# Chain123/RecGURU

Hardware: AMD Instinct MI355X
Metric: user-sequences/sec (AE+GAN step) (higher is better)
Workload: dtype bf16; 1 GPU; cross-domain RecGURU AE+GAN phase-2 iteration (5 critic + 1 generator update), two 100000-item domains; per_gpu_batch=4096, seq_len=200, d_model=128, n_head=4, n_blocks=3, d_ff=512, n_negs=30, user_lengths=U{5..220}, parallelism=dp1

## Files before the change

### include/recguru_hip.h

```cpp
#ifndef RECGURU_HIP_H
#define RECGURU_HIP_H
#include <stddef.h>
#include <stdint.h>
#ifdef __cplusplus
extern "C" {
#endif

#define RG_F32 0
#define RG_BF16 1
#define RG_X3 2

#define RG_ERR_INVALID (-1)
#define RG_ERR_UNSUPPORTED (-2)
#define RG_ERR_HIP (-3)

const char* rg_last_error(void);
int rg_version(void);

int rg_det_enabled(void);
int rg_det_set_arenas(void* fbase0, void* sbase0, unsigned long long bytes0, int bits0,
                      void* fbase1, void* sbase1, unsigned long long bytes1, int bits1);
int rg_det_fault(int clear);

#define RG_PRO_NONE 0
// ... 33 lines not shown
  const void* Y; int ldy;
  const void* X; int ldx;
  float* dW; int lddw;
  float* colsum;
  int T, N1, N2;
  int prologue_x;
  float scale;
  int splits;
  int use_tr;
  const int* live16;
  float* partials;
  int colsum_T;
} rg_gemm_tn_args;
int rg_gemm_tn(const rg_gemm_tn_args* args , int dtype, void* stream);
size_t rg_gemm_tn_workspace(const rg_gemm_tn_args* args , int dtype);
int rg_gemm_tn_layer_supported(const rg_gemm_tn_args* p , const int* wgs , int dtype);
size_t rg_gemm_tn_layer_workspace(int slot, int wgs);
int rg_gemm_tn_layer(const rg_gemm_tn_args* p , const int* wgs , int dtype, void* stream);
int rg_gemm_nt_plan(const rg_gemm_nt_args* args , int dtype, char* name, int cap);
int rg_gemm_tn_plan(const rg_gemm_tn_args* args , int dtype, char* name, int cap);


typedef struct {
  const void* qkv;
  const int64_t* key_ids; int64_t pad_value; int causal;
  void* ctx; float* lse;
  int B, L, H, dk;
  float scale;
  float drop_p; unsigned long long seed;
  const float* rowmask;
  const void* x; const void* wqkv; const float* bqkv; int d;
  int x_masked;
  const int* first_live;
  int qkv_hm;
  const void* pad_rows;
} rg_attn_args;
int rg_attn_fwd(const rg_attn_args* args , int dtype, void* stream);
int rg_attn_fwd_x_supported(int d, int dtype, float drop_p);

typedef struct {
  const void* qkv; const void* dctx; const void* ctx; const float* lse;
  const int64_t* key_ids; int64_t pad_value; int causal;
  void* dqkv;
  int B, L, H, dk;
  float scale;
  float drop_p; unsigned long long seed;
  const float* rowmask;
  const float* bqkv; int x_masked;
  const int* first_live;
  int qkv_hm;
} rg_attn_bwd_args;
int rg_attn_bwd(const rg_attn_bwd_args* args , int dtype, void* stream);

int rg_embed_pe_fwd(const void* table, const float* pe, const int64_t* ids, const float* mask, void* out,
                    long long ntok, int L, int d, float drop_p, unsigned long long seed, int dtype, void* stream);
int rg_embed_pe_fwd_rows(const void* table, long long table_rows, const float* pe, const int64_t* ids, const float* mask, void* out,
                         long long ntok, int L, int d, float drop_p, unsigned long long seed, int dtype, void* stream);
int rg_embed_pe_fwd2(const void* table, const float* pe, const int64_t* ids, const float* mask, void* out, void* out2,
                     long long ntok, int L, int d, float drop_p, unsigned long long seed, int dtype, void* stream);
int rg_embed_pe_fwd_split(const float* table_f32, const float* pe, const int64_t* ids, const float* mask, void* out,
                          void* out_lo, long long ntok, int L, int d, float drop_p, unsigned long long seed, void* stream);
int rg_embed_scatter_bwd(const void* dx, const int64_t* ids, const float* mask, float* dE, long long ntok, int d,
                         long long skip_row, float drop_p, unsigned long long seed, int dtype, void* stream);
size_t rg_embed_scatter_binned_workspace(long long ntok, int d, long long table_rows);
int rg_embed_scatter_bwd_binned(const void* dx, const int64_t* ids, const float* mask, float* dE, long long ntok, int d,
                                long long table_rows, long long skip_row, float drop_p, unsigned long long seed,
                                void* workspace, size_t workspace_bytes, int dtype, void* stream);

typedef struct {
  const void* dy; const void* y; const float* rstd; const float* gamma; const float* beta;
  const float* rowmask;
  void* dz; float* dgamma; float* dbeta;
  long long M; int N; int ld;
  void* dz_drop; float drop_p; unsigned long long drop_seed;
  const int* live16;
  float* dz_colsum;
  float* partials;
} rg_ln_bwd_args;
int rg_ln_bwd(const rg_ln_bwd_args* args , int dtype, void* stream);
size_t rg_ln_bwd_workspace(long long M, int N);

int rg_bcast_add_ln(const void* x, const float* o, const float* gamma, const float* beta, void* y, float* rstd,
                    long long M, int L, int N, float eps, int dtype, void* stream);
int rg_seq_sum(const void* x, void* out , int B, int L, int N, int dtype, void* stream);
int rg_pad_mask(const int64_t* ids, int64_t pad, float* out, long long n, void* stream);
int rg_last_rows(const void* x, const float* rowmask, void* x_last, float* m_last, int B, int L, int d, int dtype, void* stream);

int rg_colsum(const void* x, const void* aux , const float* coef , float* out,
              long long M, int N, int ld, float scale, int dtype,
              void* stream);
int rg_outer_posmask(const float* coef , const float* w , const void* aux, void* out,
                     long long M, int N, float scale, int dtype,
                     void* stream);
typedef struct {
  const void* real; const void* fake;
  const float* alpha;
  const void *W1, *W2, *W3, *W1t, *W2t, *W3t;
  const float *b1, *b2, *b3, *w4, *b4;
  int B, d, n1, n2, n3;
  float drop_p;
  unsigned long long seed_w[3];
  unsigned long long seed_g[3];
  float coef_real, coef_fake;
  float gp_coef;
  float* out;
  float* scalars;
  void *Y1, *X1, *Y2, *X2, *Y3, *X3;
  float *db1, *db2, *db3, *dw4, *db4;
  void* dx;
  void* hscratch;
  int need_wgrad;
  int debug_ablate;
  long long* stamps;
} rg_disc_args;
int rg_disc_supported(int d, int n1, int n2, int n3, int dtype);
int rg_disc_rows(const rg_disc_args* args , int dtype, void* stream);
int rg_interpolate(const float* alpha, const void* real, const void* fake, void* out, long long B, int d,
                   int dtype, void* stream);
int rg_gp_penalty(const float* g, void* dg, float* gp, long long B, int d, float lambda, int dtype,
                  void* stream);
int rg_sum(const float* x, float* out, long long n, float scale, void* stream);

int rg_adam(float* p, const float* g, float* m, float* v, void* shadow, int shadow_dtype, long long n, float lr,
            float beta1, float beta2, float eps, int step, void* stream);
typedef struct {
  float* p; const float* g; float* m; float* v;
  long long n;
  float step_lr; float inv_bc2_sqrt;
} rg_adam_seg;
int rg_adam_multi(const rg_adam_seg* segs , int nsegs, float beta1, float beta2, float eps, void* stream);
typedef struct {
  float* p; const float* g; float* m; float* v;
  long long n;
  long long step;
} rg_adam_seg_dev;
int rg_adam_multi_dev(rg_adam_seg_dev* segs , int nsegs, double lr, double beta1, double beta2,
                      double eps, void* stream);
typedef struct {
  double total_sq;
  float norm;
  float coef;
  int skip;
  int reserved;
  long long skipped;
} rg_adam_ctl;
#define RG_SQNORM_CHAIN(chunk, nsegs) \
  (((chunk) + 1023) / 1024 + 1 + 2 + 6 + 2 + 1 + (int)(((((long long)(nsegs)) + 255) / 256 + 8) >> 29))
int rg_grad_sqnorm_multi(const rg_adam_seg_dev* segs , int nsegs, float* partial ,
                         rg_adam_ctl* ctl , double max_norm, int skip_nonfinite, void* stream);
int rg_adam_multi_dev2(rg_adam_seg_dev* segs , int nsegs, double lr, double beta1, double beta2,
                       double eps, double weight_decay, int decoupled, const rg_adam_ctl* ctl , void* stream);
#define RG_CAST_TRANSPOSE 1
#define RG_CAST_PACK 2
#define RG_CAST_SPLIT 4
int rg_cast(const float* src, void* dst, int R, int C, int transpose, int dtype, void* stream);
typedef struct {
  const float* src; void* dst;
  int R, C, ld, row_off, col_off, transpose;
} rg_cast_seg;
int rg_cast_multi(const rg_cast_seg* segs , const int* tiles , int ntiles,
                  int dtype, void* stream);

#define RG_LOSS_SAMPLED_CE 0
#define RG_LOSS_BPR 1
#define RG_LOSS_BPR_SAS 2
typedef struct {
  const void* h;
// ... 94 lines not shown

typedef struct {
  const void* h;
  const void* table;
  long long first_row, n_rows;
  const int64_t* target;
  const int64_t* excl;
  const int64_t* excl_off;
  int64_t* topk_ids;
  float* topk_scores;
  int* rank;
  void* workspace; size_t workspace_bytes;
  int B, d, K;
} rg_topk_args;
size_t rg_topk_workspace(int B, int d, long long n_rows, int K);
int rg_topk_scores(const rg_topk_args* args , int dtype, void* stream);

typedef struct {
  const void* h;
  const void* table;
  long long table_rows;
  const int64_t* rows;
  long long n_list;
  const int64_t* target;
  const int64_t* excl;
  const int64_t* excl_off;
  int64_t* topk_ids;
  float* topk_scores;
  int* rank;
  void* workspace; size_t workspace_bytes;
  int B, d, K;
} rg_topk_list_args;
size_t rg_topk_list_workspace(int B, int d, long long n_list, int K);
int rg_topk_list(const rg_topk_list_args* args , int dtype, void* stream);

typedef struct {
  const void* ctx; const void* x;
  const void* Wo; const float* bo; const float* g1; const float* be1;
  const float* o_bcast; const float* gc; const float* bec; int L;
  const void* W1; const float* b1; const void* W2; const float* b2; const float* g2; const float* be2;
  const float* rowmask;
  void* out;
  void* y_save; float* rstd1; void* y2_save; float* rstd_c; void* h1_save; float* rstd2;
  int M, d, P, dff; float eps;
  float drop_p; unsigned long long seed_h1; unsigned long long seed_out;
  const float* cross_s; const float* cross_oh; const float* cross_bo; int H;
  const int* live16;
  int skip_dead_saves;
  int w_packed;
  const void* x_lo;
  void* out_lo;
} rg_post_attn_args;
int rg_post_attn_fwd(const rg_post_attn_args* args , int dtype, void* stream);

typedef struct {
  const void* dl2;
  const void* dz;
  const void* h1;
  const void* W2t;
  const void* W1t;
  void* dh1;
  void* dy;
  int M, d, dff, w_packed;
  float nz_scale;
  const int* live16;
  const void* ln_dout; const void* ln_out; const float* ln_rstd; const float* ln_gamma; const float* ln_beta;
  const float* ln_rowmask;
  void* dl2_out; float* ln_dgamma; float* ln_dbeta; float* ln_partials;
  float ln_drop_p; unsigned long long ln_drop_seed;
} rg_ffn_bwd_args;
size_t rg_ffn_bwd_ln_workspace(int M);

typedef struct {
  const void* dy; const void* y; const float* rstd; const float* gamma; const float* beta;
  const float* rowmask;
  const void* Wot;
  void* dz; void* dctx;
  float* dgamma; float* dbeta; float* ln_partials;
  int M, d, P, w_packed;
  const int* live16;
} rg_attn_out_bwd_args;
int rg_attn_out_bwd(const rg_attn_out_bwd_args* args , int dtype, void* stream);
size_t rg_attn_out_bwd_workspace(int M);
int rg_ffn_bwd_data(const rg_ffn_bwd_args* args , int dtype, void* stream);
int rg_ffn_bwd_data_supported(int d, int dff);
int rg_live_tiles(const float* rowmask, long long M, int* list, void* stream);
int rg_first_live(const float* rowmask, int B, int L, int* first, void* stream);

int rg_attn_lastq_fwd(const void* qlast, const void* kv, const int64_t* key_ids, int64_t pad_value, void* ctx,
                      int B, int L, int H, float scale, float drop_p, unsigned long long seed, int dtype, void* stream,
                      const float* bkv, const int* first_live);
int rg_attn_lastq_bwd(const void* qlast, const void* kv, const void* dctx, const int64_t* key_ids, int64_t pad_value,
                      void* dq, void* dkv, int B, int L, int H, float scale, float drop_p, unsigned long long seed,
                      int dtype, void* stream, const float* bkv, const int* first_live);

typedef struct {
  const void* x; const void* qlast; const void* wk; const void* wv;
  const float* bk; const float* bv;
  const int64_t* key_ids; int64_t pad_value;
  const int* first_live;
  void* ctx;
  const void* dctx;
  void* dx; void* dq; void* ym_v; void* ym_q; void* xbar; void* dqp; float* dbv;
  int B, L; float scale; float drop_p; unsigned long long seed;
} rg_lastq_x_args;
int rg_attn_lastq_x_supported(int d, int P, int H, int L, int dtype);
int rg_attn_lastq_x_fwd(const rg_lastq_x_args* args , void* stream);
int rg_attn_lastq_x_bwd(const rg_lastq_x_args* args , void* stream);
int rg_attn_lastq_xf_fwd(const rg_lastq_x_args* args , void* stream);
int rg_attn_lastq_xf_bwd(const rg_lastq_x_args* args , void* stream);

int rg_cross_drop_scale(const int64_t* enc_ids, int64_t pad_value, float* s, int B, int L, int H, float drop_p,
                        unsigned long long seed, void* stream);
int rg_seq_wsum(const void* x, const float* s, void* out, int B, int L, int H, int N, int dtype, void* stream);

#ifdef __cplusplus
}
#endif
#endif
```

### recguru_amd/csrc/elementwise.hip

```cpp
#include <stdlib.h>
#include "rg_common.hip.h"
#include "rg_det.hip.h"
#include "../../include/recguru_hip.h"

#define EW_BLOCK 256
static inline int ew_grid(long long work_items, int per_block) {
  long long g = (work_items + per_block - 1) / per_block;
  if (g < 1) g = 1;
  if (g > 256LL * 16) g = 256LL * 16;
  return (int)g;
}

template <typename T>
__global__ __launch_bounds__(EW_BLOCK) void embed_pe_fwd_kernel(const T* __restrict__ table, const float* __restrict__ pe,
                                                               const int64_t* __restrict__ ids,
                                                               const float* __restrict__ mask, T* __restrict__ out,
                                                               long long ntok, int L, int d, DropCfg drop) {
  const int cpr = d >> 3;
  const long long total = ntok * cpr;
  for (long long i = (long long)blockIdx.x * EW_BLOCK + threadIdx.x; i < total; i += (long long)gridDim.x * EW_BLOCK) {
    const long long tok = i / cpr;
    const int c8 = (int)(i - tok * cpr) * 8;
    const float m = mask[tok];
    const int64_t id = ids[tok];
// ... 428 lines not shown
  struct alignas(sizeof(T) * NPL) VT { T e[NPL]; };
  struct alignas(sizeof(float) * NPL) VF { float e[NPL]; };
  const int lane = threadIdx.x & 63, wave = threadIdx.x >> 6;
  const float invn = 1.f / (float)N;
  const VF g = *reinterpret_cast<const VF*>(gamma + lane * NPL), be = *reinterpret_cast<const VF*>(beta + lane * NPL);
  const long long gw = (long long)blockIdx.x * 4 + wave, nw = (long long)gridDim.x * 4;
  for (long long m = gw; m < M; m += nw) {
    const long long b = m / L;
    const VT xv = *reinterpret_cast<const VT*>(x + (size_t)m * N + lane * NPL);
    const VF ov = *reinterpret_cast<const VF*>(o + (size_t)b * N + lane * NPL);
    float v[NPL];
    float s = 0.f;
#pragma unroll
    for (int j = 0; j < NPL; ++j) {
      v[j] = (float)xv.e[j] + ov.e[j];
      s += v[j];
    }
    const float mean = wave_sum(s) * invn;
    float q = 0.f;
#pragma unroll
    for (int j = 0; j < NPL; ++j) {
      const float dd = v[j] - mean;
      q += dd * dd;
    }
    const float rstd = __builtin_amdgcn_rsqf(wave_sum(q) * invn + eps);
    VT yv;
#pragma unroll
    for (int j = 0; j < NPL; ++j) yv.e[j] = (T)((v[j] - mean) * rstd * g.e[j] + be.e[j]);
    *reinterpret_cast<VT*>(y + (size_t)m * N + lane * NPL) = yv;
    if (lane == 0) rstd_out[m] = rstd;
  }
}

template <typename T, int NPL>
__global__ __launch_bounds__(EW_BLOCK) void cross_add_ln_kernel(const T* __restrict__ x, const float* __restrict__ s,
                                                               const float* __restrict__ oh, const float* __restrict__ bo,
                                                               const float* __restrict__ gamma, const float* __restrict__ beta,
                                                               T* __restrict__ y, float* __restrict__ rstd_out, long long M, int L,
                                                               int H, float eps) {
  constexpr int N = 64 * NPL;
  struct alignas(sizeof(T) * NPL) VT { T e[NPL]; };
  struct alignas(sizeof(float) * NPL) VF { float e[NPL]; };
  const int lane = threadIdx.x & 63, wave = threadIdx.x >> 6;
  const float invn = 1.f / (float)N;
  const VF g = *reinterpret_cast<const VF*>(gamma + lane * NPL), be = *reinterpret_cast<const VF*>(beta + lane * NPL);
  const VF b0 = *reinterpret_cast<const VF*>(bo + lane * NPL);
  const long long gw = (long long)blockIdx.x * 4 + wave, nw = (long long)gridDim.x * 4;
  for (long long m = gw; m < M; m += nw) {
    const long long b = m / L;
    const VT xv = *reinterpret_cast<const VT*>(x + (size_t)m * N + lane * NPL);
    float acc[NPL];
#pragma unroll
    for (int j = 0; j < NPL; ++j) acc[j] = b0.e[j];
    for (int h = 0; h < H; ++h) {
      const float sh = s[m * H + h];
      const VF ov = *reinterpret_cast<const VF*>(oh + ((size_t)b * H + h) * N + lane * NPL);
#pragma unroll
      for (int j = 0; j < NPL; ++j) acc[j] += sh * ov.e[j];
    }
    float v[NPL];
    float sum = 0.f;
#pragma unroll
    for (int j = 0; j < NPL; ++j) {
      v[j] = (float)xv.e[j] + acc[j];
      sum += v[j];
    }
    const float mean = wave_sum(sum) * invn;
    float q = 0.f;
#pragma unroll
    for (int j = 0; j < NPL; ++j) {
      const float dd = v[j] - mean;
      q += dd * dd;
    }
    const float rstd = __builtin_amdgcn_rsqf(wave_sum(q) * invn + eps);
    VT yv;
#pragma unroll
    for (int j = 0; j < NPL; ++j) yv.e[j] = (T)((v[j] - mean) * rstd * g.e[j] + be.e[j]);
    *reinterpret_cast<VT*>(y + (size_t)m * N + lane * NPL) = yv;
    if (lane == 0) rstd_out[m] = rstd;
  }
}

template <typename T>
__global__ __launch_bounds__(EW_BLOCK) void seq_sum_kernel(const T* __restrict__ x, T* __restrict__ out, int L, int N) {
  const int b = blockIdx.x;
  for (int n = threadIdx.x; n < N; n += EW_BLOCK) {
    float s = 0.f;
    for (int t = 0; t < L; ++t) s += (float)x[((size_t)b * L + t) * N + n];
    out[(size_t)b * N + n] = (T)s;
  }
}

template <typename T>
__global__ __launch_bounds__(EW_BLOCK) void colsum_kernel(const T* __restrict__ x, const T* __restrict__ aux, const float* __restrict__ coef,
                                                         float* __restrict__ out, long long M, int N, int ld, float scale) {
  const int n = blockIdx.x * 64 + (threadIdx.x & 63);
  const int part = threadIdx.x >> 6;
  __shared__ float red[4][64];
  float s = 0.f;
  if (n < N)
    for (long long m = (long long)blockIdx.y * 4 + part; m < M; m += (long long)gridDim.y * 4) {
      float v = (float)x[(size_t)m * ld + n];
      if (aux && !((float)aux[(size_t)m * ld + n] > 0.f)) v = 0.f;
      if (coef) v *= coef[m];
      s += v;
    }
  red[part][threadIdx.x & 63] = s;
  __syncthreads();
  if (part == 0 && n < N) rg_acc(out + n, (red[0][threadIdx.x] + red[1][threadIdx.x] + red[2][threadIdx.x] + red[3][threadIdx.x]) * scale);
}

template <typename T>
__global__ __launch_bounds__(EW_BLOCK) void outer_posmask_kernel(const float* __restrict__ coef, const float* __restrict__ w,
                                                                const T* __restrict__ aux, T* __restrict__ out, long long M, int N,
                                                                float scale) {
  const long long total = M * N;
  for (long long i = (long long)blockIdx.x * EW_BLOCK + threadIdx.x; i < total; i += (long long)gridDim.x * EW_BLOCK) {
    const long long m = i / N;
    const int n = (int)(i - m * N);
    const float c = (coef ? coef[m] : 1.f) * scale;
    out[i] = (T)(((float)aux[i] > 0.f) ? c * w[n] : 0.f);
  }
}

template <typename T>
__global__ __launch_bounds__(EW_BLOCK) void interpolate_kernel(const float* __restrict__ alpha, const T* __restrict__ real,
                                                              const T* __restrict__ fake, T* __restrict__ out, long long B, int d) {
  const long long total = B * d;
  for (long long i = (long long)blockIdx.x * EW_BLOCK + threadIdx.x; i < total; i += (long long)gridDim.x * EW_BLOCK) {
    const float al = alpha[i / d];
    out[i] = (T)(al * (float)real[i] + (1.f - al) * (float)fake[i]);
  }
}

template <typename T>
__global__ __launch_bounds__(EW_BLOCK) void gp_penalty_kernel(const float* __restrict__ g, T* __restrict__ dg, float* __restrict__ gp,
                                                             long long B, int d, float lambda) {
  const int lane = threadIdx.x & 63, wave = threadIdx.x >> 6;
  const long long gw = (long long)blockIdx.x * 4 + wave, nw = (long long)gridDim.x * 4;
  float acc = 0.f;
  for (long long b = gw; b < B; b += nw) {
    float s = 0.f;
    for (int e = lane; e < d; e += 64) { const float v = g[(size_t)b * d + e]; s += v * v; }
    const float nrm = sqrtf(wave_sum(s));
    const float c = lambda * 2.f / (float)B * (nrm - 1.f) / nrm;
    for (int e = lane; e < d; e += 64) dg[(size_t)b * d + e] = (T)(c * g[(size_t)b * d + e]);
    acc += (nrm - 1.f) * (nrm - 1.f);
  }
  if (lane == 0 && acc != 0.f) rg_acc(gp, acc * lambda / (float)B);
}

__global__ __launch_bounds__(EW_BLOCK) void sum_kernel(const float* __restrict__ x, float* __restrict__ out, long long n, float scale) {
  float s = 0.f;
  for (long long i = (long long)blockIdx.x * EW_BLOCK + threadIdx.x; i < n; i += (long long)gridDim.x * EW_BLOCK) s += x[i];
  s = wave_sum(s);
  if ((threadIdx.x & 63) == 0 && s != 0.f) rg_acc(out, s * scale);
}

template <typename S>
__global__ __launch_bounds__(EW_BLOCK) void adam_kernel(float* __restrict__ p, const float* __restrict__ g, float* __restrict__ m,
                                                       float* __restrict__ v, S* __restrict__ shadow, long long n, float lr,
                                                       float b1, float b2, float eps, float bc1, float bc2_sqrt) {
  for (long long i = (long long)blockIdx.x * EW_BLOCK + threadIdx.x; i < n; i += (long long)gridDim.x * EW_BLOCK) {
    const float gi = g[i];
    const float mi = b1 * m[i] + (1.f - b1) * gi;
    const float vi = b2 * v[i] + (1.f - b2) * gi * gi;
    m[i] = mi;
    v[i] = vi;
    const float denom = sqrtf(vi) / bc2_sqrt + eps;
    const float pi = p[i] - (lr / bc1) * (mi / denom);
    p[i] = pi;
// ... 107 lines not shown
      cast_pack_tile<T>(tile, dst, r0, c0, transpose & 1, 0, 0, ((transpose & 1) ? R : C) / 32, transpose & 4);
      __syncthreads();
    }
    return;
  }
  if (!transpose) {
    const long long total = (long long)R * C;
    for (long long i = (long long)blockIdx.x * EW_BLOCK + threadIdx.x; i < total; i += (long long)gridDim.x * EW_BLOCK) dst[i] = (T)src[i];
    return;
  }
  __shared__ float tile[32][33];
  const int tx = threadIdx.x & 31, ty = threadIdx.x >> 5;
  const int tiles_c = (C + 31) / 32, tiles_r = (R + 31) / 32;
  for (int t = blockIdx.x; t < tiles_c * tiles_r; t += gridDim.x) {
    const int r0 = (t / tiles_c) * 32, c0 = (t % tiles_c) * 32;
    for (int k = ty; k < 32; k += 8) tile[k][tx] = (r0 + k < R && c0 + tx < C) ? src[(size_t)(r0 + k) * C + c0 + tx] : 0.f;
    __syncthreads();
    for (int k = ty; k < 32; k += 8)
      if (c0 + k < C && r0 + tx < R) dst[(size_t)(c0 + k) * R + r0 + tx] = (T)tile[tx][k];
    __syncthreads();
  }
}

template <typename T>
__global__ __launch_bounds__(EW_BLOCK) void cast_multi_kernel(const rg_cast_seg* __restrict__ segs, const int* __restrict__ tiles) {
  __shared__ float tile[32][33];
  const rg_cast_seg sg = segs[tiles[2 * blockIdx.x]];
  const int t = tiles[2 * blockIdx.x + 1];
  const int tx = threadIdx.x & 31, ty = threadIdx.x >> 5;
  const int tiles_c = (sg.C + 31) / 32;
  const int r0 = (t / tiles_c) * 32, c0 = (t % tiles_c) * 32;
  T* __restrict__ dst = reinterpret_cast<T*>(sg.dst);
  for (int k = ty; k < 32; k += 8) tile[k][tx] = (r0 + k < sg.R && c0 + tx < sg.C) ? sg.src[(size_t)(r0 + k) * sg.C + c0 + tx] : 0.f;
  __syncthreads();
  if (sg.transpose & 2) {
    cast_pack_tile<T>(tile, dst, r0, c0, sg.transpose & 1, sg.row_off, sg.col_off, sg.ld / 32, sg.transpose & 4);
  } else if (sg.transpose) {
    for (int k = ty; k < 32; k += 8)
      if (c0 + k < sg.C && r0 + tx < sg.R) dst[(size_t)(c0 + k + sg.row_off) * sg.ld + r0 + tx + sg.col_off] = (T)tile[tx][k];
  } else {
    for (int k = ty; k < 32; k += 8)
      if (r0 + k < sg.R && c0 + tx < sg.C) dst[(size_t)(r0 + k + sg.row_off) * sg.ld + c0 + tx + sg.col_off] = (T)tile[k][tx];
  }
}

__global__ __launch_bounds__(EW_BLOCK) void cross_drop_scale_kernel(const int64_t* __restrict__ ids, int64_t pad, float* __restrict__ s,
                                                                   int B, int L, int H, DropCfg drop) {
  __shared__ unsigned int live[64];
  __shared__ int nlive_s;
  const int b = blockIdx.x, tid = threadIdx.x;
  const unsigned int nw = rg_lpad(L) >> 5;
  if (tid < 64) live[tid] = 0u;
  if (tid == 0) nlive_s = 0;
  __syncthreads();
  for (int j = tid; j < L; j += EW_BLOCK)
    if (ids[(size_t)b * L + j] != pad) { atomicOr(&live[j >> 5], 1u << (j & 31)); atomicAdd(&nlive_s, 1); }
  __syncthreads();
  const int n = nlive_s;
  const bool all_masked = n == 0;
  if (all_masked) {
    __syncthreads();
    for (int j = tid; j < L; j += EW_BLOCK) atomicOr(&live[j >> 5], 1u << (j & 31));
    __syncthreads();
  }
  const float inv_n = 1.f / (float)(all_masked ? L : n);
  for (int i = tid; i < L * H; i += EW_BLOCK) {
    const int q = i / H, h = i - q * H;
    const unsigned int row = ((unsigned int)b * H + h) * L + q;
    float acc = 0.f;
    if (drop.onebit) {
      int cnt = 0;
      for (unsigned int w = 0; w < nw; ++w) cnt += __popc(rg_hash(drop.seed, (row * nw + w) & 0x07FFFFFFu) & live[w]);
      acc = (float)cnt * drop.inv_keep;
    } else {
      for (int j = 0; j < L; ++j)
        if ((live[j >> 5] >> (j & 31)) & 1u) acc += rg_keep(drop, row * (nw << 5) + j);
    }
    s[((size_t)b * L + q) * H + h] = acc * inv_n;
  }
}

template <typename T, int MAXH>
__global__ __launch_bounds__(EW_BLOCK) void seq_wsum_kernel(const T* __restrict__ x, const float* __restrict__ s, T* __restrict__ out,
                                                           int L, int H, int N) {
  extern __shared__ float sw_smem[];
  const int b = blockIdx.x, tid = threadIdx.x;
  const int tpr = N >> 2, rows = EW_BLOCK / tpr;
  float* sl = sw_smem;
  float* part = sw_smem + L * H;
  for (int i = tid; i < L * H; i += EW_BLOCK) sl[i] = s[(size_t)b * L * H + i];
  __syncthreads();
  const int c4 = (tid % tpr) * 4, r0 = tid / tpr;
  float acc[MAXH][4];
#pragma unroll
  for (int h = 0; h < MAXH; ++h)
#pragma unroll
    for (int j = 0; j < 4; ++j) acc[h][j] = 0.f;
  if (r0 < rows)
    for (int t = r0; t < L; t += rows) {
      float v[4];
      load4t(v, x + ((size_t)b * L + t) * N + c4);
#pragma unroll
      for (int h = 0; h < MAXH; ++h)
        if (h < H) {
          const float w = sl[t * H + h];
#pragma unroll
          for (int j = 0; j < 4; ++j) acc[h][j] += w * v[j];
        }
    }
  if (r0 < rows) {
#pragma unroll
    for (int h = 0; h < MAXH; ++h)
      if (h < H) {
#pragma unroll
        for (int j = 0; j < 4; ++j) part[((size_t)r0 * H + h) * N + c4 + j] = acc[h][j];
      }
  }
  __syncthreads();
  for (int i = tid; i < H * N; i += EW_BLOCK) {
    float t = 0.f;
    for (int r = 0; r < rows; ++r) t += part[(size_t)r * H * N + i];
    out[(size_t)b * H * N + i] = (T)t;
  }
}

__global__ __launch_bounds__(EW_BLOCK) void live_flags_kernel(const float* __restrict__ rowmask, long long M, unsigned long long* __restrict__ masks) {
  const long long nt = (M + 15) >> 4, ntp = (nt + 63) & ~63ll;
  for (long long t = (long long)blockIdx.x * EW_BLOCK + threadIdx.x; t < ntp; t += (long long)gridDim.x * EW_BLOCK) {
    int live = 0;
    if (t < nt) {
      if (16 * t + 16 <= M && (reinterpret_cast<uintptr_t>(rowmask) & 15) == 0) {
#pragma unroll
        for (int j = 0; j < 4; ++j) {
          const float4 v = reinterpret_cast<const float4*>(rowmask + 16 * t)[j];
          live |= (v.x != 0.f) | (v.y != 0.f) | (v.z != 0.f) | (v.w != 0.f);
        }
      } else {
        for (long long r = 16 * t; r < min(16 * t + 16, M); ++r) live |= rowmask[r] != 0.f;
      }
    }
    const unsigned long long m = __ballot(live != 0);
    if ((threadIdx.x & 63) == 0) masks[t >> 6] = m;
  }
}

#define LIVE_MAXW 8192
__global__ __launch_bounds__(1024) void live_compact_kernel(long long nt, int* __restrict__ list, const unsigned long long* __restrict__ masks) {
  extern __shared__ __align__(8) unsigned char live_smem[];
  const int nwords = (int)((nt + 63) >> 6);
  unsigned long long* wm = reinterpret_cast<unsigned long long*>(live_smem);
  int* woff = reinterpret_cast<int*>(live_smem + (size_t)nwords * 8);
  __shared__ int part[1024];
  const int tid = threadIdx.x, lane = tid & 63, wave = tid >> 6;
  const int per = (nwords + 1023) / 1024;
  const int w0 = min(tid * per, nwords), w1 = min(w0 + per, nwords);
  int cnt = 0;
  for (int w = w0; w < w1; ++w) { const unsigned long long m = masks[w]; wm[w] = m; cnt += __popcll(m); }
  part[tid] = cnt;
  __syncthreads();
  for (int o = 1; o < 1024; o <<= 1) {
    const int v = tid >= o ? part[tid - o] : 0;
    __syncthreads();
    part[tid] += v;
    __syncthreads();
  }
  int run = part[tid] - cnt;
  for (int w = w0; w < w1; ++w) { woff[w] = run; run += __popcll(wm[w]); }
  if (tid == 1023) list[0] = part[1023];
  __syncthreads();
  for (int w = wave; w < nwords; w += 16) {
    const long long t = 64ll * w + lane;
    const unsigned long long m = wm[w];
    const bool in = t < nt;
    const bool live = (m >> lane) & 1ull;
    const int rank = __popcll(m & ((1ull << lane) - 1ull));
    if (live) list[1 + woff[w] + rank] = (int)t;
    else if (in) list[nt - ((64ll * w - woff[w]) + (lane - rank))] = (int)t;
  }
}

template <typename T>
__global__ __launch_bounds__(EW_BLOCK) void dropout_kernel(T* __restrict__ x, long long M, int N, DropCfg drop) {
// ... 22 lines not shown
  const int n8 = N >> 3;
  const long long total = M * n8;
  for (long long i = (long long)blockIdx.x * EW_BLOCK + threadIdx.x; i < total; i += (long long)gridDim.x * EW_BLOCK) {
    const long long m = i / n8;
    const int c8 = (int)(i - m * n8) * 8;
    float v[8];
    load8(v, x + (size_t)m * N + c8);
    if (drop.thresh) {
      float k8[8];
      rg_keep8(drop, (unsigned int)m * (unsigned int)N + (unsigned int)c8, k8);
#pragma unroll
      for (int j = 0; j < 8; ++j) v[j] *= k8[j];
      store8(x + (size_t)m * N + c8, v);
    }
#pragma unroll
    for (int j = 0; j < 8; ++j) v[j] = gelu_t<PRECISE>((float)(T)v[j]);
    store8(g + (size_t)m * N + c8, v);
  }
}

template <typename T, int NPL>
__global__ __launch_bounds__(EW_BLOCK) void add_drop_ln_kernel(const T* __restrict__ x, const T* __restrict__ z,
                                                              const float* __restrict__ gamma, const float* __restrict__ beta,
                                                              const float* __restrict__ rowmask, T* __restrict__ y,
                                                              float* __restrict__ rstd_out, long long M, DropCfg drop, float eps) {
  constexpr int N = 64 * NPL;
  struct alignas(sizeof(T) * NPL) VT { T e[NPL]; };
  struct alignas(sizeof(float) * NPL) VF { float e[NPL]; };
  const int lane = threadIdx.x & 63, wave = threadIdx.x >> 6;
  const float invn = 1.f / (float)N;
  const VF g = *reinterpret_cast<const VF*>(gamma + lane * NPL), be = *reinterpret_cast<const VF*>(beta + lane * NPL);
  const long long gw = (long long)blockIdx.x * 4 + wave, nw = (long long)gridDim.x * 4;
  for (long long m = gw; m < M; m += nw) {
    const VT xv = *reinterpret_cast<const VT*>(x + (size_t)m * N + lane * NPL);
    const VT zv = *reinterpret_cast<const VT*>(z + (size_t)m * N + lane * NPL);
    const float rm = rowmask ? rowmask[m] : 1.f;
    float v[NPL];
    float s = 0.f;
#pragma unroll
    for (int j = 0; j < NPL; ++j) {
      const float k = drop.thresh ? rg_keep(drop, (unsigned int)m * (unsigned int)N + (unsigned int)(lane * NPL + j)) : 1.f;
      v[j] = (float)xv.e[j] + (float)(T)((float)zv.e[j] * k);
      s += v[j];
    }
    const float mean = wave_sum(s) * invn;
    float q = 0.f;
#pragma unroll
    for (int j = 0; j < NPL; ++j) {
      const float dd = v[j] - mean;
      q += dd * dd;
    }
    const float rstd = __builtin_amdgcn_rsqf(wave_sum(q) * invn + eps);
    VT yv;
#pragma unroll
    for (int j = 0; j < NPL; ++j) yv.e[j] = (T)(((v[j] - mean) * rstd * g.e[j] + be.e[j]) * rm);
    *reinterpret_cast<VT*>(y + (size_t)m * N + lane * NPL) = yv;
    if (lane == 0) rstd_out[m] = rstd;
  }
}

__global__ __launch_bounds__(EW_BLOCK) void cross_rows_kernel(const float* __restrict__ s, const float* __restrict__ oh,
                                                             const float* __restrict__ bo, float* __restrict__ out, long long M, int L,
                                                             int H, int N) {
  const long long total = M * N;
  for (long long i = (long long)blockIdx.x * EW_BLOCK + threadIdx.x; i < total; i += (long long)gridDim.x * EW_BLOCK) {
    const long long m = i / N;
    const int n = (int)(i - m * N);
    float acc = bo[n];
    for (int h = 0; h < H; ++h) acc += s[m * H + h] * oh[((m / L) * H + h) * N + n];
    out[i] = acc;
  }
}

extern "C" int rg_cross_drop_scale(const int64_t* enc_ids, int64_t pad_value, float* s, int B, int L, int H, float drop_p,
                                   unsigned long long seed, void* stream) {
  if (B <= 0) return 0;
  if (L > 2048) return rg_set_error_msg(RG_ERR_UNSUPPORTED, "cross_drop_scale: L > 2048");
  hipLaunchKernelGGL(cross_drop_scale_kernel, dim3(B), dim3(EW_BLOCK), 0, (hipStream_t)stream,
                     enc_ids, pad_value, s, B, L, H, make_drop(drop_p, seed));
  RG_CHECK_LAUNCH();
  return 0;
}

extern "C" int rg_seq_wsum(const void* x, const float* s, void* out, int B, int L, int H, int N, int dtype, void* stream) {
  if (B <= 0) return 0;
  hipStream_t st = (hipStream_t)stream;
  const int tpr = N >> 2;
  if ((N & 3) || tpr < 1 || tpr > EW_BLOCK || (EW_BLOCK % tpr) || H > 8)
    return rg_set_error_msg(RG_ERR_UNSUPPORTED, "seq_wsum: needs N/4 a divisor of the block size and H <= 8");
  const size_t smem = ((size_t)L * H + (size_t)(EW_BLOCK / tpr) * H * N) * sizeof(float);
  if (smem > 64 * 1024) return rg_set_error_msg(RG_ERR_UNSUPPORTED, "seq_wsum: L*H + rows*H*N floats exceed 64 KB of LDS (N = 128 / H = 4: L <= 3072; N = 256 / H = 8: L <= 1024)");
  if (dtype == RG_BF16) hipLaunchKernelGGL((seq_wsum_kernel<__bf16, 8>), dim3(B), dim3(EW_BLOCK), smem, st, (const __bf16*)x, s, (__bf16*)out, L, H, N);
  else if (dtype == RG_F32) hipLaunchKernelGGL((seq_wsum_kernel<float, 8>), dim3(B), dim3(EW_BLOCK), smem, st, (const float*)x, s, (float*)out, L, H, N);
  else return rg_set_error_msg(RG_ERR_INVALID, "seq_wsum: bad dtype");
  RG_CHECK_LAUNCH();
  return 0;
}

#define DISPATCH_T(dtype, CALL_BF16, CALL_F32, name)                                     \
  if ((dtype) == RG_BF16) { CALL_BF16; } else if ((dtype) == RG_F32) { CALL_F32; }        \
  else return rg_set_error_msg(RG_ERR_INVALID, name ": bad dtype");                       \
  RG_CHECK_LAUNCH(); return 0;

__global__ __launch_bounds__(EW_BLOCK) void first_live_kernel(const float* __restrict__ rowmask, int B, int L, int* __restrict__ first) {
  const int lane = threadIdx.x & 63, wave = threadIdx.x >> 6;
  for (int b = blockIdx.x * (EW_BLOCK / 64) + wave; b < B; b += gridDim.x * (EW_BLOCK / 64)) {
    int f = L;
    for (int l0 = 0; l0 < L && f == L; l0 += 64) {
      const int l = l0 + lane;
      const unsigned long long m = __ballot(l < L && rowmask[(size_t)b * L + l] != 0.f);
      if (m) f = l0 + __builtin_ctzll(m);
    }
    if (lane == 0) first[b] = f;
  }
}
extern "C" int rg_first_live(const float* rowmask, int B, int L, int* first, void* stream) {
  if (B <= 0 || L <= 0) return 0;
  hipLaunchKernelGGL(first_live_kernel, dim3(ew_grid((long long)B * 64, EW_BLOCK)), dim3(EW_BLOCK), 0, (hipStream_t)stream, rowmask, B, L, first);
  RG_CHECK_LAUNCH();
  return 0;
}

extern "C" int rg_live_tiles(const float* rowmask, long long M, int* list, void* stream) {
  if (M <= 0) return 0;
  const long long nt = (M + 15) >> 4;
  const int nwords = (int)((nt + 63) >> 6);
  if (nwords > LIVE_MAXW) return rg_set_error_msg(RG_ERR_UNSUPPORTED, "live_tiles: more than 8.4 M rows");
  unsigned long long* masks = reinterpret_cast<unsigned long long*>((reinterpret_cast<uintptr_t>(list + 1 + nt) + 7) & ~(uintptr_t)7);
  hipLaunchKernelGGL(live_flags_kernel, dim3(ew_grid(nt, EW_BLOCK)), dim3(EW_BLOCK), 0, (hipStream_t)stream, rowmask, M, masks);
  const int smem = nwords * 12;
  hipFuncSetAttribute(reinterpret_cast<const void*>(live_compact_kernel), hipFuncAttributeMaxDynamicSharedMemorySize, smem);
  hipLaunchKernelGGL(live_compact_kernel, dim3(1), dim3(1024), smem, (hipStream_t)stream, nt, list, masks);
  RG_CHECK_LAUNCH();
  return 0;
}

__global__ __launch_bounds__(EW_BLOCK) void pad_mask_kernel(const int64_t* __restrict__ ids, int64_t pad, float* __restrict__ out, long long n) {
  for (long long i = (long long)blockIdx.x * EW_BLOCK + threadIdx.x; i < n; i += (long long)gridDim.x * EW_BLOCK)
    out[i] = ids[i] != pad ? 1.f : 0.f;
}

template <typename T>
__global__ __launch_bounds__(EW_BLOCK) void last_rows_kernel(const T* __restrict__ x, const float* __restrict__ rowmask, T* __restrict__ x_last,
                                                            float* __restrict__ m_last, int B, int L, int d) {
  const long long total = (long long)B * d;
  for (long long i = (long long)blockIdx.x * EW_BLOCK + threadIdx.x; i < total; i += (long long)gridDim.x * EW_BLOCK) {
    const int b = (int)(i / d), c = (int)(i - (long long)b * d);
    x_last[i] = x[((size_t)b * L + L - 1) * d + c];
    if (c == 0 && m_last) m_last[b] = rowmask[(size_t)b * L + L - 1];
  }
}

extern "C" int rg_pad_mask(const int64_t* ids, int64_t pad, float* out, long long n, void* stream) {
  if (n <= 0) return 0;
  hipLaunchKernelGGL(pad_mask_kernel, dim3(ew_grid(n, EW_BLOCK)), dim3(EW_BLOCK), 0, (hipStream_t)stream, ids, pad, out, n);
  RG_CHECK_LAUNCH();
  return 0;
}

extern "C" int rg_last_rows(const void* x, const float* rowmask, void* x_last, float* m_last, int B, int L, int d, int dtype,
                            void* stream) {
  if (B <= 0 || L <= 0 || d <= 0) return 0;
  hipStream_t s = (hipStream_t)stream;
  const int grid = ew_grid((long long)B * d, EW_BLOCK);
  DISPATCH_T(dtype,
             hipLaunchKernelGGL(last_rows_kernel<__bf16>, dim3(grid), dim3(EW_BLOCK), 0, s, (const __bf16*)x, rowmask, (__bf16*)x_last, m_last, B, L, d),
             hipLaunchKernelGGL(last_rows_kernel<float>, dim3(grid), dim3(EW_BLOCK), 0, s, (const float*)x, rowmask, (float*)x_last, m_last, B, L, d),
             "last_rows")
}

extern "C" int rg_dropout(void* x, long long M, int N, float drop_p, unsigned long long seed, int dtype, void* stream) {
  if (M <= 0 || N <= 0 || drop_p <= 0.f) return 0;
  const DropCfg drop = make_drop(drop_p, seed);
  hipStream_t s = (hipStream_t)stream;
  const int grid = ew_grid(M * ((N & 7) ? N : (N >> 3)), EW_BLOCK);
  DISPATCH_T(dtype,
// ... 135 lines not shown
  if (ntok <= 0) return 0;
  if (d & 7) return rg_set_error_msg(RG_ERR_UNSUPPORTED, "embed_pe_fwd_split: d must be a multiple of 8");
  if (!table_f32 || !out || !out_lo) return rg_set_error_msg(RG_ERR_INVALID, "embed_pe_fwd_split: table_f32, out and out_lo are required");
  const int grid = ew_grid(ntok * (d >> 3), EW_BLOCK);
  hipLaunchKernelGGL(embed_pe_fwd_split_kernel, dim3(grid), dim3(EW_BLOCK), 0, (hipStream_t)stream, table_f32, pe, ids, mask,
                     (__bf16*)out, (__bf16*)out_lo, ntok, L, d, drop);
  RG_CHECK_LAUNCH();
  return 0;
}

extern "C" int rg_embed_scatter_bwd(const void* dx, const int64_t* ids, const float* mask, float* dE, long long ntok, int d,
                                    long long skip_row, float drop_p, unsigned long long seed, int dtype, void* stream) {
  const DropCfg drop = make_drop(drop_p, seed);
  if (ntok <= 0) return 0;
  hipStream_t s = (hipStream_t)stream;
  const size_t smem = (size_t)ES_SLOTS * d * sizeof(float);
  if (d > 256) return rg_set_error_msg(RG_ERR_UNSUPPORTED, "embed_scatter_bwd: d > 256");
  int grid = ew_grid(ntok, 4 * ES_UNROLL);
  const int cap = 256 * (d <= 128 ? 4 : 2);
  if (grid > cap) grid = cap;
#define RG_ES(T, NPL) hipLaunchKernelGGL((embed_scatter_bwd_kernel<T, NPL>), dim3(grid), dim3(EW_BLOCK), smem, s, (const T*)dx, ids, mask, dE, ntok, d, skip_row, drop)
#define RG_ES_T(T)                   \
  do {                               \
    if (d <= 64) RG_ES(T, 1);        \
    else if (d <= 128) RG_ES(T, 2);  \
    else RG_ES(T, 4);                \
  } while (0)
  DISPATCH_T(dtype, RG_ES_T(__bf16), RG_ES_T(float),
             "embed_scatter_bwd")
}

template <typename T>
static int launch_ln_bwd(const rg_ln_bwd_args& a, hipStream_t s) {
  const int grid = ew_grid(a.M, 64);
  if (a.N == 32) hipLaunchKernelGGL((ln_bwd_kernel<T, 4>), dim3(grid), dim3(EW_BLOCK), 0, s, a);
  else if (a.N == 64) hipLaunchKernelGGL((ln_bwd_kernel<T, 8>), dim3(grid), dim3(EW_BLOCK), 0, s, a);
  else if (a.N == 128) hipLaunchKernelGGL((ln_bwd_kernel<T, 16>), dim3(grid), dim3(EW_BLOCK), 0, s, a);
  else if (a.N == 256) hipLaunchKernelGGL((ln_bwd_kernel<T, 32>), dim3(grid), dim3(EW_BLOCK), 0, s, a);
  else return rg_set_error_msg(RG_ERR_UNSUPPORTED, "ln_bwd: N must be 32, 64, 128 or 256");
  if (a.partials && (a.dgamma || a.dbeta || a.dz_colsum))
    hipLaunchKernelGGL(ln_bwd_reduce_kernel, dim3(grid < 64 ? grid : 64), dim3(256), 0, s, a.partials, grid, a.N, a.dgamma, a.dbeta,
                       a.dz_colsum);
  RG_CHECK_LAUNCH();
  return 0;
}
extern "C" size_t rg_ln_bwd_workspace(long long M, int N) {
  return (size_t)ew_grid(M, 64) * 3 * N * sizeof(float);
}
extern "C" int rg_ln_bwd(const rg_ln_bwd_args* a, int dtype, void* stream) {
  if (!a || a->M <= 0) return 0;
  if (dtype == RG_BF16) return launch_ln_bwd<__bf16>(*a, (hipStream_t)stream);
  if (dtype == RG_F32) return launch_ln_bwd<float>(*a, (hipStream_t)stream);
  return rg_set_error_msg(RG_ERR_INVALID, "ln_bwd: bad dtype");
}

template <typename T>
static int launch_bcast_ln(const void* x, const float* o, const float* gamma, const float* beta, void* y, float* rstd,
                           long long M, int L, int N, float eps, hipStream_t s) {
  const int grid = ew_grid(M, 16);
#define RG_BV(NPL) hipLaunchKernelGGL((bcast_add_ln_vec_kernel<T, NPL>), dim3(grid), dim3(EW_BLOCK), 0, s, (const T*)x, o, gamma, beta, (T*)y, rstd, M, L, eps)
  if (N == 128 || N == 256) {
    if (N == 128) RG_BV(2); else RG_BV(4);
    RG_CHECK_LAUNCH();
    return 0;
  }
#undef RG_BV
#define RG_BL(NPL) hipLaunchKernelGGL((bcast_add_ln_kernel<T, NPL>), dim3(grid), dim3(EW_BLOCK), 0, s, (const T*)x, o, gamma, beta, (T*)y, rstd, M, L, N, eps)
  if (N <= 64) RG_BL(1);
  else if (N <= 128) RG_BL(2);
  else if (N <= 256) RG_BL(4);
  else return rg_set_error_msg(RG_ERR_UNSUPPORTED, "bcast_add_ln: N > 256");
#undef RG_BL
  RG_CHECK_LAUNCH();
  return 0;
}
extern "C" int rg_bcast_add_ln(const void* x, const float* o, const float* gamma, const float* beta, void* y, float* rstd,
                               long long M, int L, int N, float eps, int dtype, void* stream) {
  if (M <= 0) return 0;
  if (dtype == RG_BF16) return launch_bcast_ln<__bf16>(x, o, gamma, beta, y, rstd, M, L, N, eps, (hipStream_t)stream);
  if (dtype == RG_F32) return launch_bcast_ln<float>(x, o, gamma, beta, y, rstd, M, L, N, eps, (hipStream_t)stream);
  return rg_set_error_msg(RG_ERR_INVALID, "bcast_add_ln: bad dtype");
}

extern "C" int rg_seq_sum(const void* x, void* out, int B, int L, int N, int dtype, void* stream) {
  if (B <= 0) return 0;
  hipStream_t s = (hipStream_t)stream;
  DISPATCH_T(dtype,
             hipLaunchKernelGGL(seq_sum_kernel<__bf16>, dim3(B), dim3(EW_BLOCK), 0, s, (const __bf16*)x, (__bf16*)out, L, N),
             hipLaunchKernelGGL(seq_sum_kernel<float>, dim3(B), dim3(EW_BLOCK), 0, s, (const float*)x, (float*)out, L, N),
             "seq_sum")
}

extern "C" int rg_colsum(const void* x, const void* aux, const float* coef, float* out, long long M, int N, int ld, float scale,
                         int dtype, void* stream) {
  if (M <= 0) return 0;
  hipStream_t s = (hipStream_t)stream;
  long long gy = (M + 255) / 256; if (gy > 512) gy = 512; if (gy < 1) gy = 1;
  dim3 grid((N + 63) / 64, (int)gy);
  DISPATCH_T(dtype,
             hipLaunchKernelGGL(colsum_kernel<__bf16>, grid, dim3(EW_BLOCK), 0, s, (const __bf16*)x, (const __bf16*)aux, coef, out, M, N, ld, scale),
             hipLaunchKernelGGL(colsum_kernel<float>, grid, dim3(EW_BLOCK), 0, s, (const float*)x, (const float*)aux, coef, out, M, N, ld, scale),
             "colsum")
}

extern "C" int rg_outer_posmask(const float* coef, const float* w, const void* aux, void* out, long long M, int N, float scale,
                                int dtype, void* stream) {
  if (M <= 0) return 0;
  hipStream_t s = (hipStream_t)stream;
  const int grid = ew_grid(M * N, EW_BLOCK);
  DISPATCH_T(dtype,
             hipLaunchKernelGGL(outer_posmask_kernel<__bf16>, dim3(grid), dim3(EW_BLOCK), 0, s, coef, w, (const __bf16*)aux, (__bf16*)out, M, N, scale),
             hipLaunchKernelGGL(outer_posmask_kernel<float>, dim3(grid), dim3(EW_BLOCK), 0, s, coef, w, (const float*)aux, (float*)out, M, N, scale),
             "outer_posmask")
}

extern "C" int rg_interpolate(const float* alpha, const void* real, const void* fake, void* out, long long B, int d, int dtype, void* stream) {
  if (B <= 0) return 0;
  hipStream_t s = (hipStream_t)stream;
  const int grid = ew_grid(B * d, EW_BLOCK);
  DISPATCH_T(dtype,
             hipLaunchKernelGGL(interpolate_kernel<__bf16>, dim3(grid), dim3(EW_BLOCK), 0, s, alpha, (const __bf16*)real, (const __bf16*)fake, (__bf16*)out, B, d),
             hipLaunchKernelGGL(interpolate_kernel<float>, dim3(grid), dim3(EW_BLOCK), 0, s, alpha, (const float*)real, (const float*)fake, (float*)out, B, d),
             "interpolate")
}

extern "C" int rg_gp_penalty(const float* g, void* dg, float* gp, long long B, int d, float lambda, int dtype, void* stream) {
  if (B <= 0) return 0;
  hipStream_t s = (hipStream_t)stream;
  const int grid = ew_grid(B, 4);
  DISPATCH_T(dtype,
             hipLaunchKernelGGL(gp_penalty_kernel<__bf16>, dim3(grid), dim3(EW_BLOCK), 0, s, g, (__bf16*)dg, gp, B, d, lambda),
             hipLaunchKernelGGL(gp_penalty_kernel<float>, dim3(grid), dim3(EW_BLOCK), 0, s, g, (float*)dg, gp, B, d, lambda),
             "gp_penalty")
}

template <typename T>
__global__ __launch_bounds__(EW_BLOCK) void scale_dev_kernel(T* __restrict__ x, long long n8, const float* __restrict__ sp) {
  const float s = sp[0];
  if (s == 1.f) return;
  for (long long i = (long long)blockIdx.x * EW_BLOCK + threadIdx.x; i < n8; i += (long long)gridDim.x * EW_BLOCK) {
    float v[8];
    load8(v, x + 8 * i);
#pragma unroll
    for (int j = 0; j < 8; ++j) v[j] *= s;
    store8(x + 8 * i, v);
  }
}

extern "C" int rg_scale_dev(void* x, long long n, const float* s, int dtype, void* stream) {
  if (n <= 0) return 0;
  if (n % 8 || !s) return rg_set_error_msg(RG_ERR_INVALID, "scale_dev: n must be a multiple of 8 and s non-null");
  hipStream_t st = (hipStream_t)stream;
  const int grid = ew_grid(n / 8, EW_BLOCK);
  DISPATCH_T(dtype,
             hipLaunchKernelGGL(scale_dev_kernel<__bf16>, dim3(grid), dim3(EW_BLOCK), 0, st, (__bf16*)x, n / 8, s),
             hipLaunchKernelGGL(scale_dev_kernel<float>, dim3(grid), dim3(EW_BLOCK), 0, st, (float*)x, n / 8, s),
             "scale_dev")
}

template <typename T>
__global__ __launch_bounds__(EW_BLOCK) void mse_kernel(const T* __restrict__ a, const T* __restrict__ b, float* __restrict__ out,
                                                     T* __restrict__ da, T* __restrict__ db, long long n8, float inv_n) {
  float acc = 0.f;
  for (long long i = (long long)blockIdx.x * EW_BLOCK + threadIdx.x; i < n8; i += (long long)gridDim.x * EW_BLOCK) {
    float x[8], y[8], g[8];
    load8(x, a + 8 * i);
    load8(y, b + 8 * i);
#pragma unroll
    for (int j = 0; j < 8; ++j) { const float d = x[j] - y[j]; acc += d * d; g[j] = 2.f * inv_n * d; }
    if (da) store8(da + 8 * i, g);
    if (db) {
#pragma unroll
// ... 93 lines not shown
```

### recguru_amd/csrc/fused.hip

```cpp
#include <type_traits>
#include "rg_common.hip.h"
#include "rg_det.hip.h"
#include "../../include/recguru_hip.h"

#define FT_M 64
#include <stdlib.h>
#define FD 128
#define FPAD 8
#define FLD (FD + FPAD)

template <typename T> struct Tile {
  static constexpr int LD = sizeof(T) == 2 ? FD : FLD;
  static __device__ __forceinline__ int off(int row, int col) {
    if constexpr (sizeof(T) == 2) return row * FD + ((((col >> 3) ^ row) & 15) << 3) + (col & 7);
    else return row * FLD + col;
  }
};
template <> struct Tile<x3r> {
  static constexpr int LD = FD;
  static __device__ __forceinline__ int off(int row, int col) { return row * FD + ((((col >> 3) ^ row) & 15) << 3) + (col & 7); }
};

template <typename T> struct WSet { typename OpT<T>::type f[4][2]; };

// ... 1005 lines not shown
            xh[j] = ((float)xpre[i].v[j] * irm - bet[j]) * igam[j];
            g[j] = d * gam[j];
            dg[j] += d * xh[j];
            db[j] += d;
            s1 += g[j];
            s2 += g[j] * xh[j];
          }
        } else {
#pragma unroll
          for (int j = 0; j < 8; ++j) { g[j] = 0.f; xh[j] = 0.f; }
        }
#pragma unroll
        for (int o = 1; o < 16; o <<= 1) { s1 += __shfl_xor(s1, o); s2 += __shfl_xor(s2, o); }
        const float rstd = rm != 0.f ? rs_pre[i] : 0.f;
        s1 *= 1.f / FD;
        s2 *= 1.f / FD;
        float o8[8];
#pragma unroll
        for (int j = 0; j < 8; ++j) o8[j] = rstd * (g[j] - s1 - xh[j] * s2);
        store8(Adz + Tile<LT>::off(r, c8), o8);
        if (live) store8(gofs(dz, (unsigned int)(m * FD + c8)), o8);
      }
    }
    prefetch_rows(mbn);
    lds_barrier();
    f32x4 acc[2][4];
#pragma unroll
    for (int ct = 0; ct < 2; ++ct)
#pragma unroll
      for (int rt = 0; rt < 4; ++rt) acc[ct][rt] = (f32x4){0.f, 0.f, 0.f, 0.f};
    mma_wset<T>(acc, w, Adz, li, lg);
    regs_to_tile<XT>(acc, Aout, n0, li, lg);
    lds_barrier();
    tile_to_hbm<T>(Aout, dctx, FD, 0, mb, a.M, tid);
#pragma unroll
    for (int rt = 0; rt < 4; ++rt) mb[rt] = mbn[rt];
    have = have_next;
  }
#pragma unroll
  for (int o = 16; o < 64; o <<= 1)
#pragma unroll
    for (int j = 0; j < 8; ++j) { dg[j] += __shfl_xor(dg[j], o); db[j] += __shfl_xor(db[j], o); }
  float* red = reinterpret_cast<float*>(smem);
  __syncthreads();
  if (lane < 16) {
#pragma unroll
    for (int j = 0; j < 8; ++j) { red[(0 * 4 + wave) * FD + lane * 8 + j] = dg[j]; red[(1 * 4 + wave) * FD + lane * 8 + j] = db[j]; }
  }
  __syncthreads();
  const int wsel = tid >> 7, n = tid & 127;
  a.ln_partials[((size_t)blockIdx.x * 2 + wsel) * FD + n] = (red[(wsel * 4 + 0) * FD + n] + red[(wsel * 4 + 1) * FD + n]) + (red[(wsel * 4 + 2) * FD + n] + red[(wsel * 4 + 3) * FD + n]);
}

static int attn_out_bwd_grid(int M) {
  const int ntiles = (M + FT_M - 1) / FT_M;
  return ntiles < 512 ? ntiles : 512;
}
extern "C" size_t rg_attn_out_bwd_workspace(int M) { return (size_t)(M <= 0 ? 0 : 1024) * 2 * FD * sizeof(float); }

extern "C" int rg_attn_out_bwd(const rg_attn_out_bwd_args* a, int dtype, void* stream) {
  if (!a || a->M <= 0) return 0;
  if (a->d != FD || a->P != FD) return rg_set_error_msg(RG_ERR_UNSUPPORTED, "attn_out_bwd: needs d_model == n_heads*32 == 128");
  if (!a->dy || !a->y || !a->rstd || !a->gamma || !a->beta || !a->Wot || !a->dz || !a->dctx || !a->ln_partials)
    return rg_set_error_msg(RG_ERR_INVALID, "attn_out_bwd: NULL operand");
  if ((long long)a->M * FD * 4 >= (1ll << 32)) return rg_set_error_msg(RG_ERR_UNSUPPORTED, "attn_out_bwd: M too large for 32-bit offsets");
  hipStream_t s = (hipStream_t)stream;
  const int smem = 2 * act_tile_bytes(dtype, FT_M) + 3 * FD * 4;
  const int grid = attn_out_bwd_grid(a->M);
  if (dtype == RG_BF16) {
    hipFuncSetAttribute(reinterpret_cast<const void*>(attn_out_bwd_kernel<__bf16>), hipFuncAttributeMaxDynamicSharedMemorySize, smem);
    hipLaunchKernelGGL((attn_out_bwd_kernel<__bf16>), dim3(grid), dim3(256), smem, s, *a);
  } else if (dtype == RG_F32) {
    hipFuncSetAttribute(reinterpret_cast<const void*>(attn_out_bwd_kernel<float>), hipFuncAttributeMaxDynamicSharedMemorySize, smem);
    hipLaunchKernelGGL((attn_out_bwd_kernel<float>), dim3(grid), dim3(256), smem, s, *a);
  } else if (dtype == RG_X3) {
    hipFuncSetAttribute(reinterpret_cast<const void*>(attn_out_bwd_kernel<x3>), hipFuncAttributeMaxDynamicSharedMemorySize, smem);
    hipLaunchKernelGGL((attn_out_bwd_kernel<x3>), dim3(grid), dim3(256), smem, s, *a);
  } else return rg_set_error_msg(RG_ERR_INVALID, "attn_out_bwd: bad dtype");
  if (a->dgamma || a->dbeta)
    hipLaunchKernelGGL(ffn_bwd_ln_reduce_kernel, dim3(grid < 32 ? grid : 32), dim3(256), 0, s, a->ln_partials, grid, a->dgamma, a->dbeta);
  RG_CHECK_LAUNCH();
  return 0;
}
```

### recguru_amd/hip.py

```python
import ctypes
import os

import torch

_HERE = os.path.dirname(os.path.abspath(__file__))
DETERMINISTIC = os.environ.get("RG_DETERMINISTIC", "0") not in ("", "0")
LIB_PATH = os.environ.get("RG_HIP_LIB") or os.path.join(_HERE, "librecguru_hip_det.so" if DETERMINISTIC else "librecguru_hip.so")
_lib = None

F32, BF16, X3 = 0, 1, 2
SPLIT_OPERANDS = False
PRO_NONE, PRO_GELU = 0, 1
EPI_NONE, EPI_RELU, EPI_MUL_POSMASK, EPI_GELU_GRAD, EPI_ADD, EPI_RESID_LN, EPI_DROP_GELU = 0, 1, 2, 3, 4, 5, 6

c_p, c_i, c_f, c_l = ctypes.c_void_p, ctypes.c_int, ctypes.c_float, ctypes.c_int64
c_u64 = ctypes.c_uint64


class GemmNtArgs(ctypes.Structure):
    _fields_ = [("A", c_p), ("lda", c_i), ("W", c_p), ("ldw", c_i), ("bias", c_p), ("C", c_p), ("ldc", c_i),
                ("c_is_f32", c_i), ("M", c_i), ("N", c_i), ("K", c_i), ("prologue", c_i), ("epilogue", c_i),
                ("aux", c_p), ("ldaux", c_i), ("gamma", c_p), ("beta", c_p), ("rowmask", c_p),
                ("rstd_out", c_p), ("ln_eps", c_f), ("debug_ablate", c_i), ("epi_scale", c_f),
                ("epi_nonzero_scale", c_f), ("drop_p", c_f), ("drop_seed", c_u64), ("live16", c_p),
                ("skip_dead_fill", c_i), ("c_hm_L", c_i), ("C2", c_p), ("w_packed", c_i)]


class GemmTnArgs(ctypes.Structure):
    _fields_ = [("Y", c_p), ("ldy", c_i), ("X", c_p), ("ldx", c_i), ("dW", c_p), ("lddw", c_i), ("colsum", c_p),
                ("T", c_i), ("N1", c_i), ("N2", c_i), ("prologue_x", c_i), ("scale", c_f), ("splits", c_i),
                ("use_tr", c_i), ("live16", c_p), ("partials", c_p), ("colsum_T", c_i)]


class AttnArgs(ctypes.Structure):
    _fields_ = [("qkv", c_p), ("key_ids", c_p), ("pad_value", c_l), ("causal", c_i), ("ctx", c_p), ("lse", c_p),
                ("B", c_i), ("L", c_i), ("H", c_i), ("dk", c_i), ("scale", c_f), ("drop_p", c_f), ("seed", c_u64), ("rowmask", c_p),
                ("x", c_p), ("wqkv", c_p), ("bqkv", c_p), ("d", c_i), ("x_masked", c_i), ("first_live", c_p),
                ("qkv_hm", c_i), ("pad_rows", c_p)]


class AttnBwdArgs(ctypes.Structure):
    _fields_ = [("qkv", c_p), ("dctx", c_p), ("ctx", c_p), ("lse", c_p), ("key_ids", c_p), ("pad_value", c_l),
                ("causal", c_i), ("dqkv", c_p), ("B", c_i), ("L", c_i), ("H", c_i), ("dk", c_i), ("scale", c_f),
                ("drop_p", c_f), ("seed", c_u64), ("rowmask", c_p), ("bqkv", c_p), ("x_masked", c_i), ("first_live", c_p),
                ("qkv_hm", c_i)]


class PostAttnArgs(ctypes.Structure):
    _fields_ = [("ctx", c_p), ("x", c_p), ("Wo", c_p), ("bo", c_p), ("g1", c_p), ("be1", c_p),
                ("o_bcast", c_p), ("gc", c_p), ("bec", c_p), ("L", c_i),
                ("W1", c_p), ("b1", c_p), ("W2", c_p), ("b2", c_p), ("g2", c_p), ("be2", c_p),
                ("rowmask", c_p), ("out", c_p),
                ("y_save", c_p), ("rstd1", c_p), ("y2_save", c_p), ("rstd_c", c_p), ("h1_save", c_p), ("rstd2", c_p),
                ("M", c_i), ("d", c_i), ("P", c_i), ("dff", c_i), ("eps", c_f),
                ("drop_p", c_f), ("seed_h1", c_u64), ("seed_out", c_u64),
                ("cross_s", c_p), ("cross_oh", c_p), ("cross_bo", c_p), ("H", c_i), ("live16", c_p),
                ("skip_dead_saves", c_i), ("w_packed", c_i), ("x_lo", c_p), ("out_lo", c_p)]


class FfnBwdArgs(ctypes.Structure):
    _fields_ = [("dl2", c_p), ("dz", c_p), ("h1", c_p), ("W2t", c_p), ("W1t", c_p), ("dh1", c_p), ("dy", c_p),
                ("M", c_i), ("d", c_i), ("dff", c_i), ("w_packed", c_i), ("nz_scale", c_f), ("live16", c_p),
                ("ln_dout", c_p), ("ln_out", c_p), ("ln_rstd", c_p), ("ln_gamma", c_p), ("ln_beta", c_p), ("ln_rowmask", c_p),
                ("dl2_out", c_p), ("ln_dgamma", c_p), ("ln_dbeta", c_p), ("ln_partials", c_p),
                ("ln_drop_p", c_f), ("ln_drop_seed", c_u64)]


class AttnOutBwdArgs(ctypes.Structure):
    _fields_ = [("dy", c_p), ("y", c_p), ("rstd", c_p), ("gamma", c_p), ("beta", c_p), ("rowmask", c_p), ("Wot", c_p),
                ("dz", c_p), ("dctx", c_p), ("dgamma", c_p), ("dbeta", c_p), ("ln_partials", c_p),
                ("M", c_i), ("d", c_i), ("P", c_i), ("w_packed", c_i), ("live16", c_p)]


SYMBOLS = ["rg_last_error", "rg_version", "rg_gemm_nt", "rg_gemm_tn", "rg_attn_fwd", "rg_attn_bwd",
           "rg_embed_pe_fwd", "rg_embed_pe_fwd_rows", "rg_embed_scatter_bwd", "rg_ln_bwd", "rg_bcast_add_ln", "rg_seq_sum", "rg_colsum",
           "rg_outer_posmask", "rg_interpolate", "rg_gp_penalty", "rg_sum", "rg_adam", "rg_cast",
           "rg_item_loss_fwd", "rg_item_loss_bwd", "rg_post_attn_fwd",
           "rg_attn_lastq_fwd", "rg_attn_lastq_bwd",
           "rg_cross_drop_scale", "rg_seq_wsum", "rg_gemm_nt_plan", "rg_gemm_tn_plan", "rg_gemm_tn_workspace", "rg_gemm_tn_layer", "rg_gemm_tn_layer_supported", "rg_gemm_tn_layer_workspace", "rg_ln_bwd_workspace", "rg_cast_multi",
           "rg_item_loss_bwd_binned_workspace", "rg_item_loss_bwd_binned", "rg_adam_multi", "rg_rank_scores",
           "rg_assemble_batch", "rg_sample_negatives", "rg_sample_negatives_alias", "rg_dropout", "rg_cross_rows", "rg_live_tiles",
           "rg_adam_multi_dev", "rg_disc_rows", "rg_disc_supported", "rg_attn_fwd_x_supported", "rg_pad_mask", "rg_last_rows",
           "rg_ffn_bwd_data", "rg_ffn_bwd_data_supported", "rg_ffn_bwd_ln_workspace", "rg_first_live",
           "rg_attn_out_bwd", "rg_attn_out_bwd_workspace",
           "rg_item_loss_train_supported", "rg_item_loss_train", "rg_item_loss_scatter_binned", "rg_scale_dev",
           "rg_attn_lastq_x_supported", "rg_attn_lastq_x_fwd", "rg_attn_lastq_x_bwd", "rg_attn_lastq_xf_fwd", "rg_attn_lastq_xf_bwd",
           "rg_embed_scatter_binned_workspace", "rg_embed_scatter_bwd_binned", "rg_embed_pe_fwd_split", "rg_mse",
           "rg_dropout_gelu", "rg_add_drop_ln", "rg_cross_add_ln", "rg_embed_pe_fwd2",
           "rg_det_enabled", "rg_det_set_arenas", "rg_det_fault",
           "rg_full_ce_supported", "rg_full_ce_fwd", "rg_full_ce_dw",
           "rg_shared_ce_supported", "rg_shared_ce_bwd_workspace", "rg_shared_ce_fwd", "rg_shared_ce_bwd",
           "rg_topk_workspace", "rg_topk_scores", "rg_topk_list_workspace", "rg_topk_list",
           "rg_grad_sqnorm_multi", "rg_adam_multi_dev2"]
LOSS_SAMPLED_CE, LOSS_BPR, LOSS_BPR_SAS = 0, 1, 2
c_ll = ctypes.c_longlong


class LnBwdArgs(ctypes.Structure):
    _fields_ = [("dy", c_p), ("y", c_p), ("rstd", c_p), ("gamma", c_p), ("beta", c_p), ("rowmask", c_p),
                ("dz", c_p), ("dgamma", c_p), ("dbeta", c_p), ("M", c_ll), ("N", c_i), ("ld", c_i),
                ("dz_drop", c_p), ("drop_p", c_f), ("drop_seed", c_u64), ("live16", c_p), ("dz_colsum", c_p), ("partials", c_p)]


class ItemLossArgs(ctypes.Structure):
    _fields_ = [("h", c_p), ("table", c_p), ("pos", c_p), ("neg", c_p), ("mask", c_p), ("aux_tok", c_p),
                ("sums", c_p), ("gout", c_p), ("dh", c_p), ("dE", c_p), ("ntok", c_ll), ("d", c_i), ("k", c_i),
                ("mode", c_i), ("skip_row", c_ll)]


def _check_screened(path):
    if os.environ.get("RG_ALLOW_UNSCREENED") or os.environ.get("RG_HIP_LIB"):
        return
    info_path = os.path.join(_HERE, "build", "BUILD_INFO_det.json" if os.path.basename(path) == "librecguru_hip_det.so" else "BUILD_INFO.json")
    try:
        import json
        with open(info_path) as f:
            info = json.load(f)
    except (OSError, ValueError):
        return
    import hashlib
    with open(path, "rb") as f:
        sha = hashlib.sha256(f.read()).hexdigest()
    if info.get("screen_bypassed") or info.get("library_sha256") != sha:
        raise RuntimeError("recguru_amd: %s is not the library the ISA screen passed (build/BUILD_INFO.json: %s) -- rebuild with "
                           "`python -m recguru_amd.build` (RG_ALLOW_UNSCREENED=1 loads it anyway)"
                           % (path, "screen bypassed" if info.get("screen_bypassed") else "hash mismatch"))


def lib():
    global _lib
    if _lib is None:
        if not os.path.exists(LIB_PATH):
            raise RuntimeError("recguru_amd: %s is missing -- run `python -m recguru_amd.build` "
                               "(there is no CPU fallback)" % LIB_PATH)
        _check_screened(LIB_PATH)
        _lib = ctypes.CDLL(LIB_PATH)
        _lib.rg_last_error.restype = ctypes.c_char_p
        for name in SYMBOLS:
            getattr(_lib, name)
    return _lib


def _check(rc, what):
    if rc != 0:
        raise RuntimeError("%s failed (%d): %s" % (what, rc, lib().rg_last_error().decode()))


def dt_of(t):
    if t.dtype == torch.float32:
        return F32
    if t.dtype == torch.bfloat16:
        return BF16
    raise TypeError("recguru_amd: activations must be float32 or bfloat16, got %s" % t.dtype)


def mt_of(t):
    d = dt_of(t)
    return X3 if (d == F32 and SPLIT_OPERANDS) else d


def _p(t):
    if t is None:
        return None
    if not t.is_cuda:
        raise RuntimeError("recguru_amd: tensor is not on the GPU (there is no CPU path)")
    return t.data_ptr()

# ... 401 lines not shown
    ws = None
    if M >= 4096 and (dgamma is not None or dbeta is not None or dz_colsum is not None):
        fn = lib().rg_ln_bwd_workspace
        fn.restype = ctypes.c_size_t
        ws = _tn_workspace(dy.device, int(fn(c_ll(M), N)), "ln")
    a = LnBwdArgs(_p(dy), _p(y), _p(rstd), _p(gamma), _p(beta), _p(rowmask), _p(dz), _p(dgamma), _p(dbeta), M, N, N,
                  _p(dzd), drop_p, drop_seed, _p(live), _p(dz_colsum), _p(ws))
    _check(lib().rg_ln_bwd(ctypes.byref(a), dt_of(dy), _stream()), "rg_ln_bwd")
    return (dz, dzd) if drop_p > 0 else dz


def bcast_add_ln(x, o, gamma, beta, L, eps=1e-8):
    M, N = x.shape
    assert x.is_contiguous() and o.dtype == torch.float32 and o.is_contiguous()
    y = torch.empty_like(x)
    rstd = torch.empty(M, device=x.device, dtype=torch.float32)
    _check(lib().rg_bcast_add_ln(_vp(x), _vp(o), _vp(gamma), _vp(beta), _vp(y), _vp(rstd), c_ll(M), L, N,
                                 c_f(eps), dt_of(x), _stream()), "rg_bcast_add_ln")
    return y, rstd


def dropout_(x, drop_p, seed):
    assert x.is_contiguous() and x.dim() == 2
    _check(lib().rg_dropout(_vp(x), c_ll(x.shape[0]), x.shape[1], c_f(drop_p), c_u64(seed), dt_of(x), _stream()), "rg_dropout")
    return x


def dropout_gelu(x, drop_p, seed):
    assert x.is_contiguous() and x.dim() == 2
    g = torch.empty_like(x)
    _check(lib().rg_dropout_gelu(_vp(x), _vp(g), c_ll(x.shape[0]), x.shape[1], c_f(drop_p), c_u64(seed), dt_of(x), _stream()),
           "rg_dropout_gelu")
    return g


def add_drop_ln(x, z, gamma, beta, rowmask=None, drop_p=0.0, seed=0, eps=1e-8):
    M, N = x.shape
    assert x.is_contiguous() and z.is_contiguous() and z.shape == x.shape and z.dtype == x.dtype
    assert rowmask is None or (rowmask.dtype == torch.float32 and rowmask.numel() == M and rowmask.is_contiguous())
    y = torch.empty_like(x)
    rstd = torch.empty(M, device=x.device, dtype=torch.float32)
    _check(lib().rg_add_drop_ln(_vp(x), _vp(z), _vp(gamma), _vp(beta), _vp(rowmask), _vp(y), _vp(rstd), c_ll(M), N, c_f(drop_p),
                                c_u64(seed), c_f(eps), dt_of(x), _stream()), "rg_add_drop_ln")
    return y, rstd


def cross_add_ln(x, s, oh, bo, gamma, beta, L, eps=1e-8):
    M, N = x.shape
    H = s.shape[1]
    assert x.is_contiguous() and s.dtype == torch.float32 and s.is_contiguous() and s.shape[0] == M
    assert oh.dtype == torch.float32 and oh.is_contiguous() and oh.shape[1:] == (H, N)
    y = torch.empty_like(x)
    rstd = torch.empty(M, device=x.device, dtype=torch.float32)
    _check(lib().rg_cross_add_ln(_vp(x), _vp(s), _vp(oh), _vp(bo), _vp(gamma), _vp(beta), _vp(y), _vp(rstd), c_ll(M), L, H, N, c_f(eps),
                                 dt_of(x), _stream()), "rg_cross_add_ln")
    return y, rstd


def cross_rows(s, oh, bo, L):
    M, H = s.shape
    N = oh.shape[2]
    assert s.dtype == torch.float32 and oh.dtype == torch.float32 and s.is_contiguous() and oh.is_contiguous()
    out = torch.empty(M, N, device=s.device, dtype=torch.float32)
    _check(lib().rg_cross_rows(_vp(s), _vp(oh), _vp(bo), _vp(out), c_ll(M), L, H, N, _stream()), "rg_cross_rows")
    return out


def pad_mask(ids, pad):
    assert ids.dtype == torch.int64 and ids.is_contiguous()
    out = torch.empty(ids.shape, device=ids.device, dtype=torch.float32)
    _check(lib().rg_pad_mask(_vp(ids), c_l(int(pad)), _vp(out), c_ll(ids.numel()), _stream()), "rg_pad_mask")
    return out


def last_rows(x, rowmask):
    B, L, d = x.shape
    assert x.is_contiguous() and rowmask.dtype == torch.float32 and rowmask.numel() == B * L and rowmask.is_contiguous()
    xl = torch.empty(B, d, device=x.device, dtype=x.dtype)
    ml = torch.empty(B, device=x.device, dtype=torch.float32)
    _check(lib().rg_last_rows(_vp(x), _vp(rowmask), _vp(xl), _vp(ml), B, L, d, dt_of(x), _stream()), "rg_last_rows")
    return xl, ml


def seq_sum(x, B, L):
    N = x.shape[-1]
    assert x.is_contiguous()
    out = torch.empty(B, N, device=x.device, dtype=x.dtype)
    _check(lib().rg_seq_sum(_vp(x), _vp(out), B, L, N, dt_of(x), _stream()), "rg_seq_sum")
    return out


@_det_accum(out="g")
def colsum(x, out, aux=None, scale=1.0, coef=None):
    M, N = x.shape
    _check(lib().rg_colsum(_vp(x), _vp(aux), _vp(coef), _vp(out), c_ll(M), N, _rowmajor(x), c_f(scale), dt_of(x),
                           _stream()), "rg_colsum")
    return out


def outer_posmask(coef, w, aux, scale=1.0):
    M, N = aux.shape
    assert aux.is_contiguous() and w.dtype == torch.float32 and w.numel() == N
    out = torch.empty_like(aux)
    _check(lib().rg_outer_posmask(_vp(coef), _vp(w), _vp(aux), _vp(out), c_ll(M), N, c_f(scale), dt_of(aux),
                                  _stream()), "rg_outer_posmask")
    return out


def cross_drop_scale(enc_ids, pad_value, H, drop_p, seed):
    B, L = enc_ids.shape
    assert enc_ids.dtype == torch.int64 and enc_ids.is_contiguous()
    s = torch.empty(B * L, H, device=enc_ids.device, dtype=torch.float32)
    _check(lib().rg_cross_drop_scale(_vp(enc_ids), c_l(int(pad_value)), _vp(s), B, L, H, c_f(drop_p), c_u64(seed),
                                     _stream()), "rg_cross_drop_scale")
    return s


def seq_wsum(x, s, B, L, H):
    N = x.shape[-1]
    assert x.is_contiguous() and s.is_contiguous()
    out = torch.empty(B, H, N, device=x.device, dtype=x.dtype)
    _check(lib().rg_seq_wsum(_vp(x), _vp(s), _vp(out), B, L, H, N, dt_of(x), _stream()), "rg_seq_wsum")
    return out


def interpolate(alpha, real, fake):
    B, d = real.shape
    assert real.is_contiguous() and fake.is_contiguous() and alpha.dtype == torch.float32 and alpha.numel() == B
    out = torch.empty_like(real)
    _check(lib().rg_interpolate(_vp(alpha), _vp(real), _vp(fake), _vp(out), c_ll(B), d, dt_of(real), _stream()),
           "rg_interpolate")
    return out


@_det_accum(gp="s")
def gp_penalty(g, gp, lam, dtype):
    B, d = g.shape
    assert g.dtype == torch.float32 and g.is_contiguous()
    dg = torch.empty(B, d, device=g.device, dtype=dtype)
    _check(lib().rg_gp_penalty(_vp(g), _vp(dg), _vp(gp), c_ll(B), d, c_f(lam), dt_of(dg), _stream()), "rg_gp_penalty")
    return dg


@_det_accum(out="s")
def sum_into(x, out, scale=1.0):
    assert x.dtype == torch.float32 and x.is_contiguous()
    _check(lib().rg_sum(_vp(x), _vp(out), c_ll(x.numel()), c_f(scale), _stream()), "rg_sum")
    return out


def adam(p, g, m, v, shadow, lr, beta1, beta2, eps, step):
    assert p.dtype == torch.float32 and g.dtype == torch.float32 and p.is_contiguous() and g.is_contiguous()
    sd = dt_of(shadow) if shadow is not None else 0
    _check(lib().rg_adam(_vp(p), _vp(g), _vp(m), _vp(v), _vp(shadow), sd, c_ll(p.numel()), c_f(lr), c_f(beta1),
                         c_f(beta2), c_f(eps), int(step), _stream()), "rg_adam")


ADAM_CHUNK = 1 << 16
ADAM_SEG_DTYPE = [("p", "<u8"), ("g", "<u8"), ("m", "<u8"), ("v", "<u8"), ("n", "<i8"), ("step_lr", "<f4"), ("inv_bc2_sqrt", "<f4")]


def adam_multi(seg_table_dev, nsegs, beta1, beta2, eps):
    _check(lib().rg_adam_multi(_vp(seg_table_dev), int(nsegs), c_f(beta1), c_f(beta2), c_f(eps), _stream()), "rg_adam_multi")


ADAM_SEG_DEV_DTYPE = [("p", "<u8"), ("g", "<u8"), ("m", "<u8"), ("v", "<u8"), ("n", "<i8"), ("step", "<i8")]
c_d = ctypes.c_double


def adam_multi_dev(seg_table_dev, nsegs, lr, beta1, beta2, eps):
    _check(lib().rg_adam_multi_dev(_vp(seg_table_dev), int(nsegs), c_d(lr), c_d(beta1), c_d(beta2), c_d(eps), _stream()),
           "rg_adam_multi_dev")


ADAM_CTL_DTYPE = [("total_sq", "<f8"), ("norm", "<f4"), ("coef", "<f4"), ("skip", "<i4"), ("reserved", "<i4"), ("skipped", "<i8")]


def sqnorm_chain(chunk, nsegs):
    return (chunk + 1023) // 1024 + 1 + 2 + 6 + 2 + 1 + (((nsegs + 255) // 256 + 8) >> 29)


def grad_sqnorm_multi(seg_table_dev, nsegs, partial, ctl, max_norm=0.0, skip_nonfinite=False):
    assert partial is None or (partial.dtype == torch.float32 and partial.is_contiguous() and partial.numel() >= nsegs)
    assert ctl is None or (ctl.dtype == torch.uint8 and ctl.is_contiguous() and ctl.numel() >= 32)
    _check(lib().rg_grad_sqnorm_multi(_vp(seg_table_dev), int(nsegs), _vp(partial), _vp(ctl), c_d(max_norm), int(bool(skip_nonfinite)),
                                      _stream()), "rg_grad_sqnorm_multi")


def adam_multi_dev2(seg_table_dev, nsegs, lr, beta1, beta2, eps, weight_decay=0.0, decoupled=False, ctl=None):
    _check(lib().rg_adam_multi_dev2(_vp(seg_table_dev), int(nsegs), c_d(lr), c_d(beta1), c_d(beta2), c_d(eps), c_d(weight_decay),
                                    int(bool(decoupled)), _vp(ctl), _stream()), "rg_adam_multi_dev2")


CAST_SEG_DTYPE = [("src", "<u8"), ("dst", "<u8"), ("R", "<i4"), ("C", "<i4"), ("ld", "<i4"), ("row_off", "<i4"),
                  ("col_off", "<i4"), ("transpose", "<i4")]


def cast_multi(seg_table_dev, tiles_dev, ntiles, dtype):
    code = BF16 if dtype == torch.bfloat16 else F32
    _check(lib().rg_cast_multi(_vp(seg_table_dev), _vp(tiles_dev), int(ntiles), code, _stream()), "rg_cast_multi")


CAST_TRANSPOSE, CAST_PACK, CAST_SPLIT = 1, 2, 4


# ... 484 lines not shown
        return hit[1]
    flags = torch.empty(1 + 2 * ((M + 15) // 16) + 4, device=rowmask.device, dtype=torch.int32)
    _check(lib().rg_live_tiles(_vp(rowmask), c_ll(M), _vp(flags), _stream()), "rg_live_tiles")
    if len(_LIVE) >= 32:
        _LIVE.pop(next(iter(_LIVE)))
    _LIVE[key] = (rowmask, flags)
    return flags


_FIRST = {}


def first_live(rowmask, B, L):
    key = (rowmask.data_ptr(), rowmask._version, B, L)
    hit = _FIRST.get(key)
    if hit is not None:
        return hit[1]
    out = torch.empty(B, device=rowmask.device, dtype=torch.int32)
    _check(lib().rg_first_live(_vp(rowmask), B, L, _vp(out), _stream()), "rg_first_live")
    if len(_FIRST) >= 32:
        _FIRST.pop(next(iter(_FIRST)))
    _FIRST[key] = (rowmask, out)
    return out


def post_attn_fwd(ctx, x, Wo, bo, g1, be1, W1, b1, W2, b2, g2, be2, rowmask, save=False, cross=None, L=0, eps=1e-8,
                  drop_p=0.0, seed_h1=0, seed_out=0, cross_drop=None, compact=True, skip_dead_saves=False, w_packed=False,
                  x_lo=None):
    M, P = ctx.shape
    d = x.shape[1]
    dff = W1.shape[0]
    dev = ctx.device
    live16 = None
    if rowmask is not None and M >= COMPACT_MIN_ROWS and compact:
        live16 = live_tiles(rowmask, M)
    out = torch.empty(M, d, device=dev, dtype=ctx.dtype)
    sv = {}
    if save:
        sv["y"] = torch.empty(M, d, device=dev, dtype=ctx.dtype)
        sv["rstd1"] = torch.empty(M, device=dev, dtype=torch.float32)
        sv["h1"] = torch.empty(M, dff, device=dev, dtype=ctx.dtype)
        sv["rstd2"] = torch.empty(M, device=dev, dtype=torch.float32)
        if cross is not None:
            sv["y2"] = torch.empty(M, d, device=dev, dtype=ctx.dtype)
            sv["rstd_c"] = torch.empty(M, device=dev, dtype=torch.float32)
        if POISON_UNWRITTEN and live16 is not None and skip_dead_saves:
            for t in sv.values():
                t.fill_(float("nan"))
    o, gc, bec = cross if cross is not None else (None, None, None)
    cs, coh, cbo, cH = cross_drop if cross_drop is not None else (None, None, None, 0)
    out_lo = None
    if x_lo is not None:
        assert x_lo.shape == x.shape and x_lo.dtype == x.dtype == torch.bfloat16 and x_lo.is_contiguous()
        out_lo = sv["out_lo"] = torch.empty_like(out)
    a = PostAttnArgs(_p(ctx), _p(x), _p(Wo), _p(bo), _p(g1), _p(be1), _p(o), _p(gc), _p(bec), L,
                     _p(W1), _p(b1), _p(W2), _p(b2), _p(g2), _p(be2), _p(rowmask), _p(out),
                     _p(sv.get("y")), _p(sv.get("rstd1")), _p(sv.get("y2")), _p(sv.get("rstd_c")), _p(sv.get("h1")),
                     _p(sv.get("rstd2")), M, d, P, dff, eps, drop_p, seed_h1, seed_out, _p(cs), _p(coh), _p(cbo), cH,
                     _p(live16), 1 if (live16 is not None and skip_dead_saves) else 0, 1 if w_packed else 0,
                     _p(x_lo), _p(out_lo))
    _check(lib().rg_post_attn_fwd(ctypes.byref(a), mt_of(ctx), _stream()), "rg_post_attn_fwd")
    return out, sv


@_det_accum(dgamma="g", dbeta="g")
def attn_out_bwd(dy, y, rstd, gamma, beta, rowmask, dgamma, dbeta, Wot, live=None, w_packed=False):
    M, d = dy.shape
    P = d
    assert dy.is_contiguous() and y.is_contiguous() and dy.dtype == y.dtype
    dz = torch.empty_like(dy)
    dctx = torch.empty(M, P, device=dy.device, dtype=dy.dtype)
    if POISON_UNWRITTEN and live is not None:
        dz.fill_(float("nan"))
        dctx.fill_(float("nan"))
    fn = lib().rg_attn_out_bwd_workspace
    fn.restype = ctypes.c_size_t
    ws = _tn_workspace(dy.device, int(fn(M)), "attn_out_ln")
    a = AttnOutBwdArgs(_p(dy), _p(y), _p(rstd), _p(gamma), _p(beta), _p(rowmask), _p(Wot), _p(dz), _p(dctx),
                       _p(dgamma), _p(dbeta), _p(ws), M, d, P, 1 if w_packed else 0, _p(live))
    _check(lib().rg_attn_out_bwd(ctypes.byref(a), mt_of(dy), _stream()), "rg_attn_out_bwd")
    return dz, dctx


def ffn_bwd_data_supported(d, dff):
    return bool(lib().rg_ffn_bwd_data_supported(int(d), int(dff)))


def ffn_bwd_data(dl2, dz, h1, W2t, W1t, nz_scale=0.0, live=None, w_packed=False, ln=None):
    src = ln[0] if ln is not None else dl2
    M, d = src.shape
    dff = h1.shape[1]
    dh1 = torch.empty(M, dff, device=src.device, dtype=src.dtype)
    if POISON_UNWRITTEN and live is not None:
        dh1.fill_(float("nan"))
    dy = torch.empty(M, d, device=src.device, dtype=src.dtype)
    a = FfnBwdArgs(_p(dl2), _p(dz), _p(h1), _p(W2t), _p(W1t), _p(dh1), _p(dy), M, d, dff, 1 if w_packed else 0,
                   float(nz_scale), _p(live))
    dl2o, sc = None, None
    if ln is not None:
        dout, out, rstd, gamma, beta, rowmask, dgamma, dbeta, drop_p, drop_seed = ln
        if DETERMINISTIC:
            sc = _DetScope()
            dgamma, dbeta = sc.take(dgamma), sc.take(dbeta)
        assert dout.is_contiguous() and out.is_contiguous() and dout.dtype == out.dtype
        dl2o = torch.empty(M, d, device=src.device, dtype=src.dtype)
        if POISON_UNWRITTEN and live is not None:
            dl2o.fill_(float("nan"))
        fn = lib().rg_ffn_bwd_ln_workspace
        fn.restype = ctypes.c_size_t
        ws = _tn_workspace(src.device, int(fn(M)), "ffn_ln")
        a.ln_dout, a.ln_out, a.ln_rstd, a.ln_gamma, a.ln_beta, a.ln_rowmask = _p(dout), _p(out), _p(rstd), _p(gamma), _p(beta), _p(rowmask)
        a.dl2_out, a.ln_dgamma, a.ln_dbeta, a.ln_partials = _p(dl2o), _p(dgamma), _p(dbeta), _p(ws)
        a.ln_drop_p, a.ln_drop_seed = float(drop_p), int(drop_seed)
    try:
        _check(lib().rg_ffn_bwd_data(ctypes.byref(a), mt_of(src), _stream()), "rg_ffn_bwd_data")
    finally:
        if sc is not None:
            sc.commit()
    return (dh1, dy, dl2o) if ln is not None else (dh1, dy)


class Profiler(object):
    def __init__(self):
        self.records = []

    @staticmethod
    def _live_frac(ref, cache):
        if ref is None:
            return 1.0
        key = (ref.data_ptr(), ref.numel(), ref.dtype)
        if key not in cache:
            if ref.dtype == torch.int32:
                nt = (ref.numel() - 5) // 2
                cache[key] = float(ref[0]) / max(nt, 1)
            else:
                m = ref.reshape(-1)
                pad = (-m.numel()) % 16
                if pad:
                    m = torch.cat([m, m.new_zeros(pad)])
                cache[key] = float((m.view(-1, 16).abs().amax(1) > 0).float().mean())
        return cache[key]

    def summary(self):
        torch.cuda.synchronize()
        agg, cache = {}, {}
        for name, fl, by, e0, e1, ref in self.records:
            a = agg.setdefault(name, {"launches": 0, "ms": 0.0, "flops": 0.0, "bytes": 0.0, "flops_exec": 0.0, "bytes_exec": 0.0})
            a["launches"] += 1
            a["ms"] += e0.elapsed_time(e1)
            for f1, b1, r1 in (zip(fl, by, ref) if isinstance(fl, list) else ((fl, by, ref),)):
                a["flops"] += f1
                a["bytes"] += b1
                if isinstance(r1, tuple) and r1 and r1[0] == "exec":
                    a["flops_exec"] += r1[1]
                    a["bytes_exec"] += r1[2]
                    continue
                if isinstance(r1, tuple) and r1 and r1[0] == "exec_rows":
                    key = ("rows", r1[1].data_ptr(), r1[1].numel())
                    if key not in cache:
                        cache[key] = float((r1[1].reshape(-1) != 0).sum())
                    a["bytes_exec"] += cache[key] * r1[2] + r1[3]
                    continue
                lf = self._live_frac(r1, cache)
                a["flops_exec"] += f1 * lf
                a["bytes_exec"] += b1 * lf
        return agg
# ... 50 lines not shown
    else:
        B, L, P3 = qkv.shape
    return ("attn_bwd_kernel<%s>" % _tn(qkv), 10.0 * B * H * L * L * 32,
            B * L * (2 * P3 + 2 * P3 // 3) * _esize(qkv))


def _work_embed_fwd(table, pe, ids, mask, L, *a, **k):
    n, d = ids.numel(), table.shape[1]
    es = _esize(table)
    return "embed_pe_fwd_kernel", 0.0, n * d * 2 * es + n * 12, ("exec_rows", mask, d * es, n * d * es + n * 12)


def _work_item_loss(h, table, pos, neg, mask, k, mode, *a, **kw):
    n, d = h.shape
    return "item_loss_kernel", 2.0 * n * (k + 1) * d, n * (k + 2) * d * _esize(table) + n * (k + 1) * 8


def _work_post_attn(ctx, x, Wo, bo, g1, be1, W1, *a, **k):
    M, P = ctx.shape
    d, dff = x.shape[1], W1.shape[0]
    by = M * (P + 2 * d) * _esize(ctx) + (M * (d + dff) * _esize(ctx) if k.get("save") else 0)
    return ("post_attn_fwd_kernel<%s>" % _tn(ctx),
            2.0 * M * (d * P + 2 * d * dff), by)


def _work_attn_fwd_x(x, wqkv, bqkv, key_ids, pad_value, causal, H, *a, **k):
    B, L, d = x.shape
    P3 = wqkv.shape[0]
    return ("attn_fwd_kernel<bf16,x-input>", 4.0 * B * H * L * L * 32 + 2.0 * B * L * d * P3,
            B * L * (d + P3 // 3) * _esize(x) + P3 * d * _esize(x))


def _work_ffn_bwd(dl2, dz, h1, *a, **k):
    src = k["ln"][0] if k.get("ln") is not None else dl2
    M, d = src.shape
    dff = h1.shape[1]
    return ("ffn_bwd_data_kernel<%s>" % _tn(src), 4.0 * M * d * dff,
            M * ((4 if k.get("ln") is not None else 3) * d + 2 * dff) * _esize(src))


def _work_lastq_x_fwd(x, q_last, *a, **k):
    B, L, d = x.shape
    return "attn_lastq_x_fwd_kernel", B * (4 * 2.0 * L * d * 2 + 4 * 2.0 * 32 * d * 2), B * L * d * _esize(x) + 2 * B * d * _esize(x)


def _work_lastq_x_bwd(x, q_last, *a, **k):
    B, L, d = x.shape
    return "attn_lastq_x_bwd_kernel", B * (4 * 2.0 * L * d * 5 + 4 * 2.0 * 32 * d * 3), 2 * B * L * d * _esize(x) + 11 * B * d * _esize(x)


def _work_item_loss_train(h, table, pos, neg, mask, k, mode, *a, **kw):
    n, d = h.shape
    nl = float(mask.sum())
    return ("item_loss_train_rows_kernel", 4.0 * nl * (k + 1) * d,
            nl * (k + 2) * d * _esize(table) + n * d * _esize(table) + nl * (k + 1) * 12 + n * 4)


def _work_item_loss_scatter(h, table_rows, pos, neg, mask, k, coef, gout, dE, *a, **kw):
    n, d = h.shape
    nl = float(mask.sum())
    pairs = nl * (k + 1)
    return "item_loss_scatter_binned_kernel", 2.0 * pairs * d, pairs * (d * _esize(h) + 2 * 12 + 2 * 8)


def _work_gemm_tn_layer(probs):
    fl, by, refs = [], [], []
    for i, pr in enumerate(probs):
        if pr is None:
            continue
        Y, X, dW, colsum, live = pr
        T, N1, N2 = Y.shape[0], Y.shape[1], X.shape[1]
        fl.append(2.0 * T * N1 * N2)
        by.append(T * (N1 + N2) * _esize(Y) + N1 * N2 * 4)
        refs.append(live)
    x3 = any(pr is not None and pr[0].dtype == torch.float32 for pr in probs)
    return "gemm_tn_layer_x3_kernel" if x3 else "gemm_tn_layer_kernel", fl, by, refs


def _work_attn_out_bwd(dy, y, rstd, *a, **k):
    M, d = dy.shape
    return "attn_out_bwd_kernel", 2.0 * M * d * d, 4 * M * d * _esize(dy) + M * 4


def _work_ln_bwd(dy, y, rstd, *a, **k):
    M, N = dy.shape
    return "ln_bwd_kernel", 0.0, 3 * M * N * _esize(dy) + M * 4


def _work_full_ce_fwd(h, w, labels, mask, live, sums, train=True):
    n, d = h.shape
    C = w.shape[0]
    nl = float(mask.sum())
    wgs = -(-int(live[0]) // (8 * (2 if d <= 128 else 1)))
    return ("full_ce_fwd_kernel<%s,%s>" % (_tn(h), "train" if train else "infer"), 2.0 * nl * C * d * (2 if train else 1),
            wgs * C * d * _esize(w) + nl * d * _esize(h) + (n * d * _esize(h) if train else 0) + n * 16)


def _work_full_ce_dw(h, w, labels, mask, live, lse, sums, gout, dw):
    n, d = h.shape
    C = w.shape[0]
    nl = float(mask.sum())
    rows_wg = 16 * 8 * (2 if d <= 128 else 1)
    return ("full_ce_dw_kernel<%s>" % _tn(h), 4.0 * nl * C * d,
            (C / rows_wg + 1) * nl * (d * _esize(h) + 16) + C * d * (_esize(w) + 8))


def _work_shared_ce_fwd(h, table, labels, cand, mask, live, sums, train=True, cand_bias=None, pos_bias=None):
    n, d = h.shape
    C = cand.numel()
    nl = float(mask.sum())
    wgs = -(-int(live[0]) // (8 * (2 if d <= 128 else 1)))
    return ("shared_ce_fwd_kernel<%s,%s>" % (_tn(h), "train" if train else "infer"), 2.0 * nl * C * d * (2 if train else 1),
            (wgs + 2) * C * d * _esize(h) + 2 * nl * d * _esize(h) + (n * d * _esize(h) if train else 0) + n * 20)


def _work_shared_ce_dw(h, table_rows, labels, cand, mask, live, wc, lse, coef_pos, sums, gout, dE, cand_bias=None, target_route=True):
    n, d = h.shape
    C = cand.numel()
    nl = float(mask.sum())
    rows_wg = 16 * 8 * (2 if d <= 128 else 1)
    fn = lib().rg_shared_ce_bwd_workspace
    fn.restype = ctypes.c_size_t
    fn.argtypes = [c_ll, c_ll, c_i]
    return ("shared_ce_dw_kernel<%s>" % _tn(h), 4.0 * nl * C * d,
            (C / rows_wg + 1) * nl * (d * _esize(h) + 16) + 2 * int(fn(n, C, d)) + C * d * (_esize(h) + 8)
            + (2 * n * d * _esize(h) if target_route else 0))


_WORK = {"full_ce_fwd": _work_full_ce_fwd, "full_ce_dw": _work_full_ce_dw, "shared_ce_fwd": _work_shared_ce_fwd, "shared_ce_dw": _work_shared_ce_dw, "attn_out_bwd": _work_attn_out_bwd, "ln_bwd": _work_ln_bwd, "gemm_tn_layer": _work_gemm_tn_layer, "item_loss_scatter_binned": _work_item_loss_scatter, "attn_lastq_x_fwd": _work_lastq_x_fwd, "attn_lastq_x_bwd": _work_lastq_x_bwd, "item_loss_train": _work_item_loss_train,
         "ffn_bwd_data": _work_ffn_bwd, "attn_fwd_x": _work_attn_fwd_x, "post_attn_fwd": _work_post_attn, "gemm_nt": _work_gemm_nt, "gemm_tn": _work_gemm_tn, "attn_fwd": _work_attn_fwd, "attn_bwd": _work_attn_bwd,
         "embed_pe_fwd": _work_embed_fwd, "item_loss_fwd": _work_item_loss, "item_loss_bwd": _work_item_loss}
_PLAIN = ["dropout_", "cross_rows", "adam_multi", "adam_multi_dev", "adam_multi_dev2", "grad_sqnorm_multi", "disc_rows", "item_loss_bwd_binned", "embed_scatter_bwd", "bcast_add_ln", "seq_sum", "colsum", "outer_posmask", "interpolate",
          "gp_penalty", "sum_into", "adam", "cast", "attn_lastq_fwd", "attn_lastq_bwd", "cross_drop_scale", "seq_wsum",
          "embed_scatter_bwd_binned", "scale_dev", "dropout_gelu", "add_drop_ln", "mse", "cross_add_ln"]


def start_profile():
    global _PROF
    import sys
    mod = sys.modules[__name__]
    _PROF = Profiler()

    def wrap(name, fn, work):
        def timed(*a, **k):
            e0 = torch.cuda.Event(enable_timing=True)
            e1 = torch.cuda.Event(enable_timing=True)
            wk = work(*a, **k) if work else (name + "_kernel", 0.0, 0.0)
            kname, fl, by = wk[:3]
            if name in ("item_loss_fwd", "item_loss_bwd"):
                rows = "_rows" if a[0].shape[1] in (64, 128, 256) else ""
                kname = "%s%s_kernel" % (name, rows)
                if name == "item_loss_bwd":
                    fl = fl * 2
            global _PLAN_NAME
            _PLAN_NAME = None
            e0.record()
            out = fn(*a, **k)
            e1.record()
            if _PLAN_NAME is not None:
                kname = _PLAN_NAME
            ref = k.get("live")
            if ref is None:
                ref = k.get("rowmask")
            if ref is None and name == "post_attn_fwd" and len(a) > 12:
                ref = a[12]
                if ref is not None and (a[0].shape[0] < COMPACT_MIN_ROWS or not k.get("compact", True)):
                    ref = None
            if ref is None and name == "ln_bwd" and len(a) > 5 and k.get("live") is None:
                ref = None
            if len(wk) > 3:
                ref = wk[3]
            _PROF.records.append((kname, fl, by, e0, e1, ref))
            return out
        return timed
    for name in list(_WORK) + _PLAIN:
        _ORIG[name] = getattr(mod, name)
        setattr(mod, name, wrap(name, _ORIG[name], _WORK.get(name)))
    return _PROF


def stop_profile():
    global _PROF
    import sys
    mod = sys.modules[__name__]
    for name, fn in _ORIG.items():
        setattr(mod, name, fn)
    _ORIG.clear()
    p, _PROF = _PROF, None
    return p
```

### recguru_amd/ops.py

```python
import os
import weakref

import torch

from . import hip

_COMPUTE = torch.bfloat16
LN_EPS = 1e-8
GP_LAMBDA = 0.1


def set_compute_dtype(dt):
    global _COMPUTE, _MIXED
    _MIXED = dt == "mixed"
    x3 = dt in ("bf16x3", "mixed")
    if x3:
        dt = torch.float32
    elif dt == "bf16":
        dt = torch.bfloat16
    elif dt == "f32":
        dt = torch.float32
    assert dt in (torch.float32, torch.bfloat16)
    _COMPUTE = dt
    hip.SPLIT_OPERANDS = x3
# ... 417 lines not shown
        else:
            out = hip.embed_pe_fwd(shadow(table), pe, ids, mask, L, drop_p, seed)
        ctx.save_for_backward(ids, mask)
        ctx.table = table
        ctx.meta = (skip_row, drop_p, seed)
        return out.view(B, L, -1)

    @staticmethod
    def backward(ctx, dx):
        ids, mask = ctx.saved_tensors
        skip_row, drop_p, seed = ctx.meta
        dE, ret = _gt(ctx.table)
        dx2 = dx.contiguous().view(-1, dx.shape[-1])
        binned = (EMBED_SCATTER_BINNED and dx2.shape[0] >= 65536
                  and hip.embed_scatter_binned_supported(dx2.shape[0], dx2.shape[1], dE.shape[0]))
        (hip.embed_scatter_bwd_binned if binned else hip.embed_scatter_bwd)(dx2, ids, mask, dE, skip_row, drop_p, seed)
        return ret, None, None, None, None, None


def embed_pe(table, pe, ids, mask, skip_row=-1, drop_p=0.0):
    out = EmbedPE.run(table, pe, ids, mask, skip_row, float(drop_p))
    out._rg_masked = (weakref.ref(mask), mask._version, out._version)
    return out


def masked_by(x, rowmask):
    tag = getattr(x, "_rg_masked", None)
    ok = (rowmask is not None and tag is not None and tag[0]() is rowmask and tag[1] == rowmask._version
          and tag[2] == x._version)
    if ok and _DEBUG:
        m = rowmask.reshape(x.shape[0], x.shape[1], 1).to(x.dtype)
        assert float((x.detach() * (1 - m)).abs().max()) == 0.0, "masked_by: a padded row of x is not zero"
    return ok


WS_SPLIT_K_DX = True
WS_PROJ_PLUS_LN = True
WS_DROP_GELU_EPILOGUE = True
_ZERO_ROWS = {}


def _zero_row(n, dev):
    key = (n, str(dev))
    z = _ZERO_ROWS.get(key)
    if z is None:
        z = _ZERO_ROWS[key] = torch.zeros(1, n, device=dev, dtype=torch.float32)
    return z


def _ws_tier():
    return _COMPUTE == torch.bfloat16 or (hip.SPLIT_OPERANDS and WS_WIDE_X3)


WS_WIDE_X3 = True


def _fusable(x2, Wo, W1):
    return hip.post_attn_supported(x2.shape[1], Wo.shape[1], W1.shape[0], x2.dtype, M=x2.shape[0]) and not (x2.shape[1] == 256 and _split_resid())


def _lo_in(x2, rows=None):
    if not _split_resid():
        return None
    lo = _LO_IN
    if lo is None:
        return torch.zeros_like(x2)
    lo = rows(lo) if rows is not None else lo
    return lo.contiguous().view(x2.shape)


def _lo_out(sv, shape):
    global _LO_OUT
    lo = sv.pop("out_lo", None)
    if lo is not None:
        _LO_OUT = lo.view(shape)


QKV_BIAS_ROWS_IN_ATTENTION = True
QKV_HEAD_MAJOR = True
QKV_HEAD_MAJOR_TRAIN = True
EMBED_SCATTER_BINNED = True
FUSE_ITEM_LOSS_TRAIN = True
FUSE_ATTN_OUT_BWD = True
LASTQ_FROM_X = True
LASTQ_FOLD_PREFIX = True
ATTN_RESIDENT_MAX_L = 416


def _zero_rows_live(rowmask, M, x_masked, K=128, N=384):
    if not x_masked or rowmask is None or not _lists_ok() or M < max(hip.COMPACT_MIN_ROWS, 4096):
        return None
    if not ((K == 128 and N in (128, 256, 384, 512)) or (K in (256, 384, 512) and N % 128 == 0 and 128 <= N <= 1024)):
        return None
    return hip.live_tiles(rowmask, M)


def _qkv_attn_fwd(x2, B, L, key_ids, pad_value, causal, H, Wq, bq, Wk, bk, Wv, bv, need_grad, drop_p=0.0, seed=0,
                  rowmask=None, x_masked=False, allow_unwritten=False):
    wqkv = shadow_cat((Wq, Wk, Wv))
    bqkv = bias_cat((bq, bk, bv))
    if not need_grad and FUSE_QKV_INFERENCE and L <= ATTN_RESIDENT_MAX_L and hip.attn_fwd_x_supported(x2.shape[1], _COMPUTE, drop_p):
        ctx_ = hip.attn_fwd_x(x2.view(B, L, -1), wqkv, bqkv, key_ids, pad_value, causal, H, drop_p=drop_p, seed=seed,
                              rowmask=rowmask, x_masked=x_masked and rowmask is not None)
        return None, ctx_, None
    live = _zero_rows_live(rowmask, x2.shape[0], x_masked, x2.shape[1], wqkv.shape[0])
    sub = live is not None and QKV_BIAS_ROWS_IN_ATTENTION and allow_unwritten and _unwritten_qkv_ok() and L <= ATTN_RESIDENT_MAX_L
    if (QKV_HEAD_MAJOR and _COMPUTE == torch.bfloat16 and (H, x2.shape[1]) in ((4, 128), (8, 256)) and x2.shape[0] >= 4096
            and 16 <= L <= ATTN_RESIDENT_MAX_L and (not need_grad or QKV_HEAD_MAJOR_TRAIN)):
        qkv = hip.gemm_nt(x2, wqkv, bqkv, live=live, skip_dead_fill=1 if sub else 2, headmajor_L=L)
        ctx_, lse = hip.attn_fwd(qkv, key_ids, pad_value, causal, H, need_lse=need_grad, drop_p=drop_p, seed=seed, rowmask=rowmask,
                                 x_masked=x_masked, bqkv=bqkv if sub else None, pad_rows=pad_rows_cat((bq, bk, bv), H))
        return qkv, ctx_, lse
    qkv = hip.gemm_nt(x2, wqkv, bqkv, live=live, skip_dead_fill=1 if sub else 2)
    ctx_, lse = hip.attn_fwd(qkv.view(B, L, -1), key_ids, pad_value, causal, H, need_lse=need_grad, drop_p=drop_p, seed=seed,
                             rowmask=rowmask, x_masked=x_masked, bqkv=bqkv if sub else None)
    return qkv, ctx_, lse


def _attn_block_fwd(x2, B, L, key_ids, pad_value, causal, H, Wq, bq, Wk, bk, Wv, bv, Wo, bo, g, be, need_grad,
                    drop_p=0.0, seed=0, rowmask=None, x_masked=False):
    qkv, ctx_, lse = _qkv_attn_fwd(x2, B, L, key_ids, pad_value, causal, H, Wq, bq, Wk, bk, Wv, bv, need_grad, drop_p, seed,
                                   rowmask, x_masked)
    M, d = x2.shape
    P = Wo.shape[1]
    if (WS_PROJ_PLUS_LN and _ws_tier() and M >= 4096 and d % 128 == 0 and P % 128 == 0 and d > 128
            and P // 128 <= 4 and d // 128 <= 8):
        lf = _live(rowmask, M, LISTS_256 and d == 256 and P == 256)
        z = hip.gemm_nt(ctx_.view(B * L, -1), shadow(Wo), bo.detach(), epilogue=hip.EPI_ADD, aux=x2, live=lf)
        y, rstd = hip.bcast_add_ln(z, _zero_row(d, z.device), g.detach(), be.detach(), M, LN_EPS)
        return y, (qkv, ctx_, lse, rstd)
    rstd = torch.empty(x2.shape[0], device=x2.device, dtype=torch.float32)
    y = hip.gemm_nt(ctx_.view(B * L, -1), shadow(Wo), bo.detach(), epilogue=hip.EPI_RESID_LN, aux=x2,
                    gamma=g.detach(), beta=be.detach(), rstd_out=rstd, eps=LN_EPS)
    return y, (qkv, ctx_, lse, rstd)


def _attn_block_bwd(dy, x2, y, saved, B, L, key_ids, pad_value, causal, H, prm, drop_p=0.0, seed=0, rowmask=None,
                    x_masked=False):
    Wq, bq, Wk, bk, Wv, bv, Wo, bo, g, be = prm
    qkv, ctx_, lse, rstd = saved
    d = x2.shape[1]
    P = Wo.shape[1]
    (dg, rg), (dbe, rbe) = _gt(g), _gt(be)
    live = _live(rowmask, dy.shape[0], (d == 128 and P == 128) or (LISTS_256 and d == 256 and P == 256 and _ws_tier()))
    (dWo, rWo), (dbo, rbo) = _gt(Wo), _gt(bo)
    if FUSE_ATTN_OUT_BWD and d == 128 and P == 128:
        dz, dctx = hip.attn_out_bwd(dy, y, rstd, g.detach(), be.detach(), rowmask, dg, dbe,
                                    shadow(Wo, transpose=True, pack=True, split=True), live=live, w_packed=True)
        _tn(dz, ctx_.view(B * L, P), dWo, dbo, live=live)
    else:
        dz = hip.ln_bwd(dy, y, rstd, g.detach(), be.detach(), rowmask, dg, dbe, live=live)
        hip.gemm_tn(dz, ctx_.view(B * L, P), dWo, dbo, live=live if live is not None else _live_tn(rowmask, dz.shape[0], P, d))
        dctx = hip.gemm_nt(dz, shadow(Wo, transpose=True), live=live, skip_dead_fill=True)
    sub = (QKV_BIAS_ROWS_IN_ATTENTION and x_masked == 2 and _unwritten_qkv_ok() and L <= ATTN_RESIDENT_MAX_L
           and _zero_rows_live(rowmask, x2.shape[0], True, d, 3 * P) is not None)
    dqkv = hip.attn_bwd(qkv if qkv.dim() == 5 else qkv.view(B, L, -1), dctx.view(B, L, P), ctx_, lse, key_ids, pad_value, causal, H,
                        drop_p=drop_p, seed=seed, rowmask=rowmask, bqkv=bias_cat((bq, bk, bv)) if sub else None)
    dqkv2 = dqkv.view(B * L, 3 * P)
    (dWqkv, rW), (dbqkv, rb) = _gt_cat((Wq, Wk, Wv)), _gt_cat((bq, bk, bv))
    _tn(dqkv2, x2, dWqkv, dbqkv)
    Wt = shadow_cat((Wq, Wk, Wv), transpose=True)
    if (WS_SPLIT_K_DX and _ws_tier() and dqkv2.shape[0] >= 4096 and 3 * P == 768 and d % 128 == 0
            and 128 < d <= 1024):
        dx = hip.gemm_nt(dqkv2[:, :384], Wt[:, :384], epilogue=hip.EPI_ADD, aux=dz, live=live)
        dx = hip.gemm_nt(dqkv2[:, 384:], Wt[:, 384:], epilogue=hip.EPI_ADD, aux=dx, out=dx, live=live)
    else:
        dx = hip.gemm_nt(dqkv2, Wt, epilogue=hip.EPI_ADD, aux=dz, live=live)
    return dx, (rW[0], rb[0], rW[1], rb[1], rW[2], rb[2], rWo, rbo, rg, rbe)


def _ffn_block_fwd(y, rowmask, W1, b1, W2, b2, g, be, drop_p=0.0, seed_h1=0, seed_out=0):
    M, d = y.shape
    dff = W1.shape[0]
    wide = WS_PROJ_PLUS_LN and _ws_tier() and M >= 4096 and d == 256 and dff % 128 == 0 and dff // 128 <= 4
    if wide and WS_DROP_GELU_EPILOGUE:
        gact = torch.empty(M, dff, device=y.device, dtype=y.dtype)
        h1 = hip.gemm_nt(y, shadow(W1), b1.detach(), epilogue=hip.EPI_DROP_GELU, drop_p=drop_p, drop_seed=seed_h1, out2=gact)
        lf = _live(rowmask, M, LISTS_256 and dff == 512)
        l2 = hip.gemm_nt(gact, shadow(W2), b2.detach(), live=lf)
        out, rstd = hip.add_drop_ln(y, l2, g.detach(), be.detach(), rowmask, drop_p, seed_out, LN_EPS)
        return out, (h1, rstd)
    h1 = hip.gemm_nt(y, shadow(W1), b1.detach())
    if wide:
        gact = hip.dropout_gelu(h1, drop_p, seed_h1)
        l2 = hip.gemm_nt(gact, shadow(W2), b2.detach())
        out, rstd = hip.add_drop_ln(y, l2, g.detach(), be.detach(), rowmask, drop_p, seed_out, LN_EPS)
        return out, (h1, rstd)
    if drop_p > 0:
        hip.dropout_(h1, drop_p, seed_h1)
        l2 = hip.gemm_nt(h1, shadow(W2), b2.detach(), prologue=hip.PRO_GELU, out_f32=True)
        hip.dropout_(l2, drop_p, seed_out)
        out, rstd = hip.bcast_add_ln(y, l2, g.detach(), be.detach(), 1, LN_EPS)
        if rowmask is not None:
            out = out * rowmask.to(out.dtype).unsqueeze(1)
        return out, (h1, rstd)
    rstd = torch.empty(y.shape[0], device=y.device, dtype=torch.float32)
    out = hip.gemm_nt(h1, shadow(W2), b2.detach(), prologue=hip.PRO_GELU, epilogue=hip.EPI_RESID_LN, aux=y,
                      gamma=g.detach(), beta=be.detach(), rowmask=rowmask, rstd_out=rstd, eps=LN_EPS)
    return out, (h1, rstd)


FUSE_FFN_BWD = True
FUSE_FFN_BWD_LN = True


def _ffn_block_bwd(dout, y, out, saved, rowmask, prm, drop_p=0.0, seed_h1=0, seed_out=0):
    W1, b1, W2, b2, g, be = prm
    h1, rstd = saved
    d, dff = W2.shape
    live = _live(rowmask, dout.shape[0], (d == 128 and dff == 512) or (LISTS_256 and d == 256 and dff == 512 and _ws_tier()))
    (dg, rg), (dbe, rbe) = _gt(g), _gt(be)
    (dW2, rW2), (db2, rb2) = _gt(W2), _gt(b2)
    (dW1, rW1), (db1, rb1) = _gt(W1), _gt(b1)
    if FUSE_FFN_BWD and FUSE_FFN_BWD_LN and hip.ffn_bwd_data_supported(d, dff):
        dh1, dy, dl2 = hip.ffn_bwd_data(None, None, h1, shadow(W2, transpose=True, pack=True, split=True), shadow(W1, transpose=True, pack=True, split=True),
                                        nz_scale=_inv_keep(drop_p), live=live, w_packed=True,
                                        ln=(dout, out, rstd, g.detach(), be.detach(), rowmask, dg, dbe, drop_p, seed_out))
        _tn(dl2, h1, dW2, db2, prologue_x=hip.PRO_GELU, live=live)
        _tn(dh1, y, dW1, db1, live=live)
        return dy, (rW1, rb1, rW2, rb2, rg, rbe)
    if drop_p > 0:
        dz, dl2 = hip.ln_bwd(dout, out, rstd, g.detach(), be.detach(), rowmask, dg, dbe, drop_p, seed_out, live=live)
    else:
        dz = dl2 = hip.ln_bwd(dout, out, rstd, g.detach(), be.detach(), rowmask, dg, dbe, live=live)
    live_tn = live if live is not None else _live_tn(rowmask, dout.shape[0], d, dff)
    hip.gemm_tn(dl2, h1, dW2, db2, prologue_x=hip.PRO_GELU, live=live_tn)
    if FUSE_FFN_BWD and hip.ffn_bwd_data_supported(d, dff):
        dh1, dy = hip.ffn_bwd_data(dl2, dz, h1, shadow(W2, transpose=True, pack=True, split=True), shadow(W1, transpose=True, pack=True, split=True),
                                   nz_scale=_inv_keep(drop_p), live=live, w_packed=True)
        hip.gemm_tn(dh1, y, dW1, db1, live=live)
        return dy, (rW1, rb1, rW2, rb2, rg, rbe)
    dh1 = hip.gemm_nt(dl2, shadow(W2, transpose=True), epilogue=hip.EPI_GELU_GRAD, aux=h1,
                      epi_nonzero_scale=_inv_keep(drop_p), live=live, skip_dead_fill=True)
    hip.gemm_tn(dh1, y, dW1, db1, live=live_tn)
    dy = hip.gemm_nt(dh1, shadow(W1, transpose=True), epilogue=hip.EPI_ADD, aux=dz, live=live)
    return dy, (rW1, rb1, rW2, rb2, rg, rbe)


class EncoderLayerFn(_Fn):

    @staticmethod
    def forward(ctx, x, key_ids, rowmask, pad_value, causal, H, drop_p,
                Wq, bq, Wk, bk, Wv, bv, Wo, bo, g1, be1, W1, b1, W2, b2, g2, be2):
        B, L, d = x.shape
        need = _needs_grad(ctx)
        x2 = x.contiguous().view(B * L, d)
        key_ids = key_ids.contiguous()
        rowmask = rowmask.reshape(-1).contiguous()
        seeds = (_draw(), _draw(), _draw()) if drop_p > 0 else (0, 0, 0)
        xm = _X_MASKED
        if _fusable(x2, Wo, W1):
# ... 150 lines not shown
                cWv, cbv, cWo, cbo, cg, cbe,
                W1, b1, W2, b2, g2, be2):
        B, L, d = x.shape
        need = _needs_grad(ctx)
        x2 = x.contiguous().view(B * L, d)
        key_ids = key_ids.contiguous()
        rowmask = rowmask.reshape(-1).contiguous()
        ctx.u_dtype = u.dtype
        u = u.to(x.dtype).contiguous()
        seeds = (_draw(), _draw(), _draw(), _draw()) if drop_p > 0 else (0, 0, 0, 0)
        P = cWv.shape[0]
        c = hip.gemm_nt(u, shadow(cWv), cbv.detach())
        s_cross = None
        if drop_p > 0:
            s_cross = hip.cross_drop_scale(enc_ids.contiguous(), 0, H, drop_p, seeds[3])
            cm = (c.view(B, 1, H, 32) * _head_eye(H, c)).view(B * H, P)
            oh = hip.gemm_nt(cm, shadow(cWo), None, out_f32=True).view(B, H, d)
            cross_kw = dict(cross=(None, cg.detach(), cbe.detach()), cross_drop=(s_cross, oh, cbo.detach(), H))
        else:
            o = hip.gemm_nt(c, shadow(cWo), cbo.detach(), out_f32=True)
            cross_kw = dict(cross=(o, cg.detach(), cbe.detach()))
        if _fusable(x2, Wo, W1):
            unw = d == 128
            qkv, ctx_, lse = _qkv_attn_fwd(x2, B, L, key_ids, 0, True, H, Wq, bq, Wk, bk, Wv, bv, need, drop_p, seeds[0],
                                           rowmask, _X_MASKED, allow_unwritten=unw)
            xm_d = (2 if _X_MASKED else 0) if unw else (1 if _X_MASKED else 0)
            out, sv = hip.post_attn_fwd(ctx_.view(B * L, -1), x2, shadow(Wo, pack=True, split=True), bo.detach(), g1.detach(), be1.detach(),
                                        shadow(W1, pack=True, split=True), b1.detach(), shadow(W2, pack=True, split=True), b2.detach(), g2.detach(),
                                        be2.detach(),
                                        rowmask, w_packed=True, save=need, L=L, eps=LN_EPS, drop_p=drop_p, seed_h1=seeds[1],
                                        seed_out=seeds[2], skip_dead_saves=_lists_everywhere(W1, B * L), x_lo=_lo_in(x2), **cross_kw)
            _lo_out(sv, (B, L, d))
            if need:
                y1, y2, rstd_c = sv["y"], sv["y2"], sv["rstd_c"]
                sa, sf = (qkv, ctx_, lse, sv["rstd1"]), (sv["h1"], sv["rstd2"])
        else:
            xm_d = 1 if _X_MASKED else 0
            y1, sa = _attn_block_fwd(x2, B, L, key_ids, 0, True, H, Wq, bq, Wk, bk, Wv, bv, Wo, bo, g1, be1, need,
                                     drop_p, seeds[0], rowmask, _X_MASKED)
            if drop_p > 0:
                if d in (128, 256):
                    y2, rstd_c = hip.cross_add_ln(y1, s_cross, oh, cbo.detach(), cg.detach(), cbe.detach(), L, LN_EPS)
                else:
                    o_rows = hip.cross_rows(s_cross, oh, cbo.detach(), L)
                    y2, rstd_c = hip.bcast_add_ln(y1, o_rows, cg.detach(), cbe.detach(), 1, LN_EPS)
            else:
                y2, rstd_c = hip.bcast_add_ln(y1, o, cg.detach(), cbe.detach(), L, LN_EPS)
            out, sf = _ffn_block_fwd(y2, rowmask, W1, b1, W2, b2, g2, be2, drop_p, seeds[1], seeds[2])
        ctx.mixed = _MIXED
        if need:
            extra = (s_cross,) if s_cross is not None else ()
            if _MIXED:
                ctx.save_for_backward(_b16(x2), _b16(u), key_ids, rowmask, _b16(y1), _b16(y2), _b16(out), _b16(c), rstd_c,
                                      _b16(sa[0]), _b16(sa[1]), sa[2], sa[3], _b16(sf[0]), sf[1], *extra)
                xm_d = 1 if xm_d else 0
            else:
                ctx.save_for_backward(x2, u, key_ids, rowmask, y1, y2, out, c, rstd_c, *sa, *sf, *extra)
            ctx.prm = (Wq, bq, Wk, bk, Wv, bv, Wo, bo, g1, be1, cWv, cbv, cWo, cbo, cg, cbe, W1, b1, W2, b2, g2, be2)
            ctx.meta = (B, L, H, drop_p, seeds, xm_d)
        return out.view(B, L, d)

    @staticmethod
    def backward(ctx, dout):
        if ctx.mixed:
            with _bf16_backward():
                return DecoderLayerFn._backward(ctx, dout.to(torch.bfloat16))
        return DecoderLayerFn._backward(ctx, dout)

    @staticmethod
    def _backward(ctx, dout):
        B, L, H, drop_p, seeds, xm = ctx.meta
        sav = ctx.saved_tensors
        x2, u, key_ids, rowmask, y1, y2, out, c, rstd_c, qkv, ctx_, lse, rstd1, h1, rstd2 = sav[:15]
        s_cross = sav[15] if len(sav) > 15 else None
        cWv, cbv, cWo, cbo, cg, cbe = ctx.prm[10:16]
        d = x2.shape[1]
        P = cWv.shape[0]
        dev = dout.device
        with _tn_layer():
            dy2, gf = _ffn_block_bwd(dout.contiguous().view(B * L, d), y2, out, (h1, rstd2), rowmask, ctx.prm[16:],
                                     drop_p, seeds[1], seeds[2])
            (dcg, rcg), (dcbe, rcbe) = _gt(cg), _gt(cbe)
            (dcWo, rcWo), (dcbo, rcbo) = _gt(cWo), _gt(cbo)
            dy1 = hip.ln_bwd(dy2, y2, rstd_c, cg.detach(), cbe.detach(), rowmask, dcg, dcbe,
                             dz_colsum=dcbo if s_cross is not None else None)
            if s_cross is None:
                do = hip.seq_sum(dy1, B, L)
                hip.gemm_tn(do, c, dcWo, dcbo)
                dc = hip.gemm_nt(do, shadow(cWo, transpose=True))
            else:
                doh = hip.seq_wsum(dy1, s_cross, B, L, H)
                eye = _head_eye(H, c)
                cm = (c.view(B, 1, H, 32) * eye).view(B * H, P)
                doh2 = doh.reshape(B * H, d)
                hip.gemm_tn(doh2, cm, dcWo)
                full = hip.gemm_nt(doh2, shadow(cWo, transpose=True))
                dc = (full.view(B, H, H, 32) * eye).sum(1).view(B, P)
            (dcWv, rcWv), (dcbv, rcbv) = _gt(cWv), _gt(cbv)
            hip.gemm_tn(dc, u, dcWv, dcbv)
            du = hip.gemm_nt(dc, shadow(cWv, transpose=True))
            dx, ga = _attn_block_bwd(dy1, x2, y1, (qkv, ctx_, lse, rstd1), B, L, key_ids, 0, True, H,
                                     ctx.prm[:10], drop_p, seeds[0], rowmask, xm)
        return ((dx.view(B, L, d), du.to(ctx.u_dtype), None, None, None, None, None) + ga + (rcWv, rcbv, rcWo, rcbo, rcg, rcbe) + gf)


class ItemLoss(_Fn):
    @staticmethod
    def forward(ctx, h, table, pos, neg, mask, k, mode, skip_row):
        d = h.shape[-1]
        h2 = h.contiguous().view(-1, d)
        pos = pos.contiguous().view(-1)
        neg = neg.contiguous().view(-1)
        mask = mask.reshape(-1).contiguous()
        tab = shadow(table)
        ctx.table = table
        ctx.meta = (k, mode, skip_row, h.shape)
        ntok = h2.shape[0]
        ctx.binned = ntok >= 65536 and bool(hip.item_loss_bwd_binned_supported(ntok, k, d, table.shape[0]))
        form = hip.item_loss_train_supported(k, d) if (FUSE_ITEM_LOSS_TRAIN and _needs_grad(ctx) and ctx.binned) else 0
        ctx.fused = form == 1 or (form == 2 and mode == hip.LOSS_SAMPLED_CE)
        ctx.lse = None
        if ctx.fused:
            sums = torch.zeros(2, device=h2.device, dtype=torch.float32)
            hip.sum_into(mask, sums[1:2])
            if _DP is not None and _DP.world > 1:
                _DP.global_count(sums[1:2])
            if form == 2:
                ctx.lse = torch.empty(ntok, device=h2.device, dtype=torch.float32)
            coef, dh1 = hip.item_loss_train(h2, tab, pos, neg, mask, k, mode, sums, lse=ctx.lse)
            ctx.save_for_backward(h2, pos, neg, mask, coef, dh1, sums)
            ctx.consumed = False
            return sums[0] / sums[1]
        sums, aux = hip.item_loss_fwd(h2, tab, pos, neg, mask, k, mode)
        if _DP is not None and _DP.world > 1:
            _DP.global_count(sums[1:2])
        ctx.save_for_backward(h2, pos, neg, mask, aux, sums)
        return sums[0] / sums[1]

    @staticmethod
    def backward(ctx, gout):
        table = ctx.table
        k, mode, skip_row, shape = ctx.meta
        dE, ret = _gt(table)
        g1 = gout.reshape(1).to(torch.float32).contiguous()
        if ctx.fused:
            h2, pos, neg, mask, coef, dh1, sums = ctx.saved_tensors
            if not ctx.consumed:
                ctx.consumed = True
                hip.item_loss_scatter_binned(h2, table.shape[0], pos, neg, mask, k, coef, g1, dE, skip_row,
                                             lse=ctx.lse, sums=sums if ctx.lse is not None else None)
                return hip.scale_dev(dh1, g1).view(shape), ret, None, None, None, None, None, None
            cnt = sums[1:2].clone()
            sums, aux = hip.item_loss_fwd(h2, shadow(table), pos, neg, mask, k, mode)
            sums[1:2] = cnt
        else:
            h2, pos, neg, mask, aux, sums = ctx.saved_tensors
        fn = hip.item_loss_bwd_binned if ctx.binned else hip.item_loss_bwd
        dh = fn(h2, shadow(table), pos, neg, mask, k, mode, aux, sums, g1, dE, skip_row)
        return dh.view(shape), ret, None, None, None, None, None, None


def sampled_softmax_loss(h, table, pos, neg, mask, k, skip_row=-1):
    return ItemLoss.run(h, table, pos, neg, mask, k, hip.LOSS_SAMPLED_CE, skip_row)


def bpr_loss(h, table, pos, neg, mask, k, skip_row=-1, sas=False):
    return ItemLoss.run(h, table, pos, neg, mask, k, hip.LOSS_BPR_SAS if sas else hip.LOSS_BPR, skip_row)


class FullSoftmaxLoss(_Fn):

    @staticmethod
    def forward(ctx, h, weight, labels, mask):
        d = h.shape[-1]
        h2 = h.contiguous().view(-1, d)
        n = h2.shape[0]
        labels = labels.contiguous().view(-1)
        mask = mask.reshape(-1).contiguous()
        if not hip.full_ce_supported(d, h2):
            raise RuntimeError("full softmax loss: no kernel for d_model=%d in the %s tier (csrc/full_ce.hip: d in 64, 128, 256)"
                               % (d, compute_tier()))
        sums = torch.zeros(2, device=h2.device, dtype=torch.float32)
        hip.sum_into(mask, sums[1:2])
        if _DP is not None and _DP.world > 1:
            _DP.global_count(sums[1:2])
# ... 265 lines not shown
```

Before: 868,300 user-sequences/sec.

## Fuse cross-attention LN backward with self-attention out-proj backward in decoder

Adds a fused kernel that runs the cross-attention LayerNorm backward, the self-attention post-LN backward and the output-projection data GEMM in one pass over live row tiles. It also accumulates the LN parameter gradients through per-block partials. This replaces separate ln_bwd and attn_out_bwd launches in the decoder backward and avoids re-reading dy1 and dz from HBM. Because the fused kernel leaves dead rows of dy1 unwritten, seq_sum and seq_wsum gain a rowmask argument so they skip padded rows. The decoder backward is split so the QKV part can be reused after the fused step.

```diff
diff --git a/include/recguru_hip.h b/include/recguru_hip.h
--- a/include/recguru_hip.h
+++ b/include/recguru_hip.h
@@ -139,7 +139,7 @@
 
 int rg_bcast_add_ln(const void* x, const float* o, const float* gamma, const float* beta, void* y, float* rstd,
                     long long M, int L, int N, float eps, int dtype, void* stream);
-int rg_seq_sum(const void* x, void* out , int B, int L, int N, int dtype, void* stream);
+int rg_seq_sum(const void* x, void* out , int B, int L, int N, int dtype, void* stream, const float* rowmask);
 int rg_pad_mask(const int64_t* ids, int64_t pad, float* out, long long n, void* stream);
 int rg_last_rows(const void* x, const float* rowmask, void* x_last, float* m_last, int B, int L, int d, int dtype, void* stream);
 
@@ -400,6 +400,18 @@
 } rg_attn_out_bwd_args;
 int rg_attn_out_bwd(const rg_attn_out_bwd_args* args , int dtype, void* stream);
 size_t rg_attn_out_bwd_workspace(int M);
+typedef struct {
+  const void* dy2; const void* y2; const float* rstd_c; const float* cgamma; const float* cbeta;
+  const void* y1; const float* rstd1; const float* gamma1; const float* beta1;
+  const float* rowmask;
+  const void* Wot;
+  void* dy1; void* dz; void* dctx;
+  float* dcgamma; float* dcbeta; float* dz_colsum; float* dgamma1; float* dbeta1; float* partials;
+  int M, d, P, w_packed;
+  const int* live16;
+} rg_attn_out_bwd_cross_args;
+int rg_attn_out_bwd_cross(const rg_attn_out_bwd_cross_args* args , int dtype, void* stream);
+size_t rg_attn_out_bwd_cross_workspace(int M);
 int rg_ffn_bwd_data(const rg_ffn_bwd_args* args , int dtype, void* stream);
 int rg_ffn_bwd_data_supported(int d, int dff);
 int rg_live_tiles(const float* rowmask, long long M, int* list, void* stream);
@@ -430,7 +442,7 @@
 
 int rg_cross_drop_scale(const int64_t* enc_ids, int64_t pad_value, float* s, int B, int L, int H, float drop_p,
                         unsigned long long seed, void* stream);
-int rg_seq_wsum(const void* x, const float* s, void* out, int B, int L, int H, int N, int dtype, void* stream);
+int rg_seq_wsum(const void* x, const float* s, void* out, int B, int L, int H, int N, int dtype, void* stream, const float* rowmask);
 
 #ifdef __cplusplus
 }
diff --git a/recguru_amd/csrc/elementwise.hip b/recguru_amd/csrc/elementwise.hip
--- a/recguru_amd/csrc/elementwise.hip
+++ b/recguru_amd/csrc/elementwise.hip
@@ -534,11 +534,15 @@
 }
 
 template <typename T>
-__global__ __launch_bounds__(EW_BLOCK) void seq_sum_kernel(const T* __restrict__ x, T* __restrict__ out, int L, int N) {
+__global__ __launch_bounds__(EW_BLOCK) void seq_sum_kernel(const T* __restrict__ x, T* __restrict__ out, int L, int N,
+                                                          const float* __restrict__ rowmask) {
   const int b = blockIdx.x;
   for (int n = threadIdx.x; n < N; n += EW_BLOCK) {
     float s = 0.f;
-    for (int t = 0; t < L; ++t) s += (float)x[((size_t)b * L + t) * N + n];
+    for (int t = 0; t < L; ++t) {
+      if (rowmask && rowmask[(size_t)b * L + t] == 0.f) continue;
+      s += (float)x[((size_t)b * L + t) * N + n];
+    }
     out[(size_t)b * N + n] = (T)s;
   }
 }
@@ -812,13 +816,16 @@
 
 template <typename T, int MAXH>
 __global__ __launch_bounds__(EW_BLOCK) void seq_wsum_kernel(const T* __restrict__ x, const float* __restrict__ s, T* __restrict__ out,
-                                                           int L, int H, int N) {
+                                                           int L, int H, int N, const float* __restrict__ rowmask) {
   extern __shared__ float sw_smem[];
   const int b = blockIdx.x, tid = threadIdx.x;
   const int tpr = N >> 2, rows = EW_BLOCK / tpr;
   float* sl = sw_smem;
   float* part = sw_smem + L * H;
+  float* ml = part + rows * H * N;
   for (int i = tid; i < L * H; i += EW_BLOCK) sl[i] = s[(size_t)b * L * H + i];
+  if (rowmask)
+    for (int i = tid; i < L; i += EW_BLOCK) ml[i] = rowmask[(size_t)b * L + i];
   __syncthreads();
   const int c4 = (tid % tpr) * 4, r0 = tid / tpr;
   float acc[MAXH][4];
@@ -828,6 +835,7 @@
     for (int j = 0; j < 4; ++j) acc[h][j] = 0.f;
   if (r0 < rows)
     for (int t = r0; t < L; t += rows) {
+      if (rowmask && ml[t] == 0.f) continue;
       float v[4];
       load4t(v, x + ((size_t)b * L + t) * N + c4);
 #pragma unroll
@@ -1016,16 +1024,17 @@
   return 0;
 }
 
-extern "C" int rg_seq_wsum(const void* x, const float* s, void* out, int B, int L, int H, int N, int dtype, void* stream) {
+extern "C" int rg_seq_wsum(const void* x, const float* s, void* out, int B, int L, int H, int N, int dtype, void* stream,
+                           const float* rowmask) {
   if (B <= 0) return 0;
   hipStream_t st = (hipStream_t)stream;
   const int tpr = N >> 2;
   if ((N & 3) || tpr < 1 || tpr > EW_BLOCK || (EW_BLOCK % tpr) || H > 8)
     return rg_set_error_msg(RG_ERR_UNSUPPORTED, "seq_wsum: needs N/4 a divisor of the block size and H <= 8");
-  const size_t smem = ((size_t)L * H + (size_t)(EW_BLOCK / tpr) * H * N) * sizeof(float);
-  if (smem > 64 * 1024) return rg_set_error_msg(RG_ERR_UNSUPPORTED, "seq_wsum: L*H + rows*H*N floats exceed 64 KB of LDS (N = 128 / H = 4: L <= 3072; N = 256 / H = 8: L <= 1024)");
-  if (dtype == RG_BF16) hipLaunchKernelGGL((seq_wsum_kernel<__bf16, 8>), dim3(B), dim3(EW_BLOCK), smem, st, (const __bf16*)x, s, (__bf16*)out, L, H, N);
-  else if (dtype == RG_F32) hipLaunchKernelGGL((seq_wsum_kernel<float, 8>), dim3(B), dim3(EW_BLOCK), smem, st, (const float*)x, s, (float*)out, L, H, N);
+  const size_t smem = ((size_t)L * H + (size_t)(EW_BLOCK / tpr) * H * N + (rowmask ? (size_t)L : 0)) * sizeof(float);
+  if (smem > 64 * 1024) return rg_set_error_msg(RG_ERR_UNSUPPORTED, "seq_wsum: L*H + rows*H*N (+ L with a row mask) floats exceed 64 KB of LDS (N = 128 / H = 4: L <= 3072; N = 256 / H = 8: L <= 1024)");
+  if (dtype == RG_BF16) hipLaunchKernelGGL((seq_wsum_kernel<__bf16, 8>), dim3(B), dim3(EW_BLOCK), smem, st, (const __bf16*)x, s, (__bf16*)out, L, H, N, rowmask);
+  else if (dtype == RG_F32) hipLaunchKernelGGL((seq_wsum_kernel<float, 8>), dim3(B), dim3(EW_BLOCK), smem, st, (const float*)x, s, (float*)out, L, H, N, rowmask);
   else return rg_set_error_msg(RG_ERR_INVALID, "seq_wsum: bad dtype");
   RG_CHECK_LAUNCH();
   return 0;
@@ -1327,12 +1336,12 @@
   return rg_set_error_msg(RG_ERR_INVALID, "bcast_add_ln: bad dtype");
 }
 
-extern "C" int rg_seq_sum(const void* x, void* out, int B, int L, int N, int dtype, void* stream) {
+extern "C" int rg_seq_sum(const void* x, void* out, int B, int L, int N, int dtype, void* stream, const float* rowmask) {
   if (B <= 0) return 0;
   hipStream_t s = (hipStream_t)stream;
   DISPATCH_T(dtype,
-             hipLaunchKernelGGL(seq_sum_kernel<__bf16>, dim3(B), dim3(EW_BLOCK), 0, s, (const __bf16*)x, (__bf16*)out, L, N),
-             hipLaunchKernelGGL(seq_sum_kernel<float>, dim3(B), dim3(EW_BLOCK), 0, s, (const float*)x, (float*)out, L, N),
+             hipLaunchKernelGGL(seq_sum_kernel<__bf16>, dim3(B), dim3(EW_BLOCK), 0, s, (const __bf16*)x, (__bf16*)out, L, N, rowmask),
+             hipLaunchKernelGGL(seq_sum_kernel<float>, dim3(B), dim3(EW_BLOCK), 0, s, (const float*)x, (float*)out, L, N, rowmask),
              "seq_sum")
 }
 
diff --git a/recguru_amd/csrc/fused.hip b/recguru_amd/csrc/fused.hip
--- a/recguru_amd/csrc/fused.hip
+++ b/recguru_amd/csrc/fused.hip
@@ -1111,3 +1111,299 @@
   RG_CHECK_LAUNCH();
   return 0;
 }
+
+template <typename T>
+__global__ __launch_bounds__(256, 2) void attn_out_bwd_cross_kernel(rg_attn_out_bwd_cross_args a) {
+  constexpr int PL = FT_M * FD * 2;
+  constexpr bool PRE_Y1 = sizeof(T) == 2;
+  typedef typename LdsT<T, PL>::type LT;
+  constexpr int ACT_BYTES = FT_M * Tile<LT>::LD * (int)sizeof(LT) * LdsT<T, PL>::PLANES;
+  extern __shared__ __align__(16) unsigned char smem[];
+  LT* Adz = reinterpret_cast<LT*>(smem);
+  typedef typename ResT<T, PL>::type XT;
+  XT* Aout = reinterpret_cast<XT*>(smem + ACT_BYTES);
+  float* lnp = reinterpret_cast<float*>(smem + 2 * ACT_BYTES);
+  float* cacc = lnp + 6 * FD;
+  const int tid = threadIdx.x, lane = tid & 63, wave = __builtin_amdgcn_readfirstlane(tid >> 6);
+  const int li = lane & 15, lg = lane >> 4;
+  const T* __restrict__ dy2 = reinterpret_cast<const T*>(a.dy2);
+  const T* __restrict__ y2 = reinterpret_cast<const T*>(a.y2);
+  const T* __restrict__ y1 = reinterpret_cast<const T*>(a.y1);
+  T* __restrict__ dy1 = reinterpret_cast<T*>(a.dy1);
+  T* __restrict__ dz = reinterpret_cast<T*>(a.dz);
+  T* __restrict__ dctx = reinterpret_cast<T*>(a.dctx);
+  const int n0 = wave * 32;
+  const int ntiles = (a.M + FT_M - 1) / FT_M;
+  for (int i = tid; i < FD; i += 256) {
+    lnp[i] = a.cgamma[i]; lnp[FD + i] = a.cbeta[i]; lnp[2 * FD + i] = 1.f / a.cgamma[i];
+    lnp[3 * FD + i] = a.gamma1[i]; lnp[4 * FD + i] = a.beta1[i]; lnp[5 * FD + i] = 1.f / a.gamma1[i];
+  }
+  WSet<T> w;
+  load_wset(w, reinterpret_cast<const T*>(a.Wot), FD, n0, 0, li, lg, a.w_packed);
+  Frag<T> cpre[4], xpre[4], ypre[4];
+  auto& yrow = [&]() -> Frag<T> (&)[4] { if constexpr (PRE_Y1) return ypre; else return xpre; }();
+  float rsc_pre[4], rs1_pre[4], rm_pre[4];
+  float dcg[8], dcb[8], dcs[8], dg[8], db[8];
+#pragma unroll
+  for (int j = 0; j < 8; ++j) { dcg[j] = 0.f; dcb[j] = 0.f; dcs[j] = 0.f; dg[j] = 0.f; db[j] = 0.f; }
+  LiveWalk lw;
+  lw.init(a.live16, a.M);
+  const int nwork = a.live16 ? (lw.nlive + 3) >> 2 : ntiles;
+  int cur = (int)blockIdx.x, kcur = 0;
+  auto next_group = [&](int (&g)[4]) -> bool {
+    if (cur >= nwork) {
+#pragma unroll
+      for (int rt = 0; rt < 4; ++rt) g[rt] = a.M;
+      return false;
+    }
+    if (!a.live16) {
+#pragma unroll
+      for (int rt = 0; rt < 4; ++rt) g[rt] = cur * FT_M + 16 * rt;
+    } else {
+      lw.group(kcur, g, a.M);
+    }
+    cur += gridDim.x;
+    ++kcur;
+    return true;
+  };
+  auto fetch_y1 = [&](const int (&g)[4]) {
+#pragma unroll
+    for (int i = 0; i < 4; ++i) {
+      const int c8 = (tid & 15) * 8, m = min(g[i] + (tid >> 4), a.M - 1);
+      load_frag(yrow[i], gofs(y1, (unsigned int)(m * FD + c8)));
+      rs1_pre[i] = a.rstd1[m];
+    }
+  };
+  auto prefetch_rows = [&](const int (&g)[4]) {
+    const float* __restrict__ rmp = a.rowmask ? a.rowmask : a.rstd_c;
+#pragma unroll
+    for (int i = 0; i < 4; ++i) {
+      const int c8 = (tid & 15) * 8, m = min(g[i] + (tid >> 4), a.M - 1);
+      load_frag(cpre[i], gofs(dy2, (unsigned int)(m * FD + c8)));
+      load_frag(xpre[i], gofs(y2, (unsigned int)(m * FD + c8)));
+      const float rv = rmp[m];
+      rsc_pre[i] = a.rstd_c[m];
+      rm_pre[i] = a.rowmask ? rv : 1.f;
+    }
+    if constexpr (PRE_Y1) fetch_y1(g);
+  };
+  int mb[4], mbn[4];
+  bool have = next_group(mb);
+  if (have) prefetch_rows(mb);
+  if constexpr (!PRE_Y1) {
+    if (lane < 16) {
+#pragma unroll
+      for (int q = 0; q < 3; ++q) store8(cacc + (q * 4 + wave) * FD + lane * 8, dcs);
+    }
+  }
+  __syncthreads();
+  for (; have;) {
+    const bool have_next = next_group(mbn);
+    const int c8 = (tid & 15) * 8;
+    {
+      float gam[8], bet[8], igam[8];
+      load8(gam, lnp + c8);
+      load8(bet, lnp + FD + c8);
+      load8(igam, lnp + 2 * FD + c8);
+#pragma unroll
+      for (int i = 0; i < 4; ++i) {
+        const int m = mb[i] + (tid >> 4);
+        const bool live = m < a.M;
+        const float rm = live ? rm_pre[i] : 0.f;
+        float g[8], xh[8], s1 = 0.f, s2 = 0.f;
+        if (rm != 0.f) {
+          const float irm = 1.f / rm;
+#pragma unroll
+          for (int j = 0; j < 8; ++j) {
+            const float d = (float)cpre[i].v[j] * rm;
+            xh[j] = ((float)xpre[i].v[j] * irm - bet[j]) * igam[j];
+            g[j] = d * gam[j];
+            dcg[j] += d * xh[j];
+            dcb[j] += d;
+            s1 += g[j];
+            s2 += g[j] * xh[j];
+          }
+        } else {
+#pragma unroll
+          for (int j = 0; j < 8; ++j) { g[j] = 0.f; xh[j] = 0.f; }
+        }
+#pragma unroll
+        for (int o = 1; o < 16; o <<= 1) { s1 += __shfl_xor(s1, o); s2 += __shfl_xor(s2, o); }
+        const float rstd = rm != 0.f ? rsc_pre[i] : 0.f;
+        s1 *= 1.f / FD;
+        s2 *= 1.f / FD;
+#pragma unroll
+        for (int j = 0; j < 8; ++j) {
+          const float o = rstd * (g[j] - s1 - xh[j] * s2);
+          dcs[j] += o;
+          cpre[i].v[j] = (T)o;
+        }
+        if (live) {
+          if constexpr (sizeof(T) == 2) *reinterpret_cast<Frag<T>*>(gofs(dy1, (unsigned int)(m * FD + c8))) = cpre[i];
+          else store8(gofs(dy1, (unsigned int)(m * FD + c8)), cpre[i].v);
+        }
+      }
+    }
+    if constexpr (!PRE_Y1) {
+      fetch_y1(mb);
+#pragma unroll
+      for (int o = 16; o < 64; o <<= 1)
+#pragma unroll
+        for (int j = 0; j < 8; ++j) { dcg[j] += __shfl_xor(dcg[j], o); dcb[j] += __shfl_xor(dcb[j], o); dcs[j] += __shfl_xor(dcs[j], o); }
+      if (lane < 16) {
+        float t[8];
+        load8(t, cacc + (0 * 4 + wave) * FD + c8);
+#pragma unroll
+        for (int j = 0; j < 8; ++j) t[j] += dcg[j];
+        store8(cacc + (0 * 4 + wave) * FD + c8, t);
+        load8(t, cacc + (1 * 4 + wave) * FD + c8);
+#pragma unroll
+        for (int j = 0; j < 8; ++j) t[j] += dcb[j];
+        store8(cacc + (1 * 4 + wave) * FD + c8, t);
+        load8(t, cacc + (2 * 4 + wave) * FD + c8);
+#pragma unroll
+        for (int j = 0; j < 8; ++j) t[j] += dcs[j];
+        store8(cacc + (2 * 4 + wave) * FD + c8, t);
+      }
+#pragma unroll
+      for (int j = 0; j < 8; ++j) { dcg[j] = 0.f; dcb[j] = 0.f; dcs[j] = 0.f; }
+    }
+    {
+      float gam[8], bet[8], igam[8];
+      load8(gam, lnp + 3 * FD + c8);
+      load8(bet, lnp + 4 * FD + c8);
+      load8(igam, lnp + 5 * FD + c8);
+#pragma unroll
+      for (int i = 0; i < 4; ++i) {
+        const int r = 16 * i + (tid >> 4), m = mb[i] + (tid >> 4);
+        const bool live = m < a.M;
+        const float rm = live ? rm_pre[i] : 0.f;
+        float g[8], xh[8], s1 = 0.f, s2 = 0.f;
+        if (rm != 0.f) {
+          const float irm = 1.f / rm;
+#pragma unroll
+          for (int j = 0; j < 8; ++j) {
+            const float d = (float)cpre[i].v[j] * rm;
+            xh[j] = ((float)yrow[i].v[j] * irm - bet[j]) * igam[j];
+            g[j] = d * gam[j];
+            dg[j] += d * xh[j];
+            db[j] += d;
+            s1 += g[j];
+            s2 += g[j] * xh[j];
+          }
+        } else {
+#pragma unroll
+          for (int j = 0; j < 8; ++j) { g[j] = 0.f; xh[j] = 0.f; }
+        }
+#pragma unroll
+        for (int o = 1; o < 16; o <<= 1) { s1 += __shfl_xor(s1, o); s2 += __shfl_xor(s2, o); }
+        const float rstd = rm != 0.f ? rs1_pre[i] : 0.f;
+        s1 *= 1.f / FD;
+        s2 *= 1.f / FD;
+        float o8[8];
+#pragma unroll
+        for (int j = 0; j < 8; ++j) o8[j] = rstd * (g[j] - s1 - xh[j] * s2);
+        store8(Adz + Tile<LT>::off(r, c8), o8);
+        if (live) store8(gofs(dz, (unsigned int)(m * FD + c8)), o8);
+      }
+    }
+    prefetch_rows(mbn);
+    lds_barrier();
+    f32x4 acc[2][4];
+#pragma unroll
+    for (int ct = 0; ct < 2; ++ct)
+#pragma unroll
+      for (int rt = 0; rt < 4; ++rt) acc[ct][rt] = (f32x4){0.f, 0.f, 0.f, 0.f};
+    mma_wset<T>(acc, w, Adz, li, lg);
+    regs_to_tile<XT>(acc, Aout, n0, li, lg);
+    lds_barrier();
+    tile_to_hbm<T>(Aout, dctx, FD, 0, mb, a.M, tid);
+#pragma unroll
+    for (int rt = 0; rt < 4; ++rt) mb[rt] = mbn[rt];
+    have = have_next;
+  }
+#pragma unroll
+  for (int o = 16; o < 64; o <<= 1)
+#pragma unroll
+    for (int j = 0; j < 8; ++j) {
+      if constexpr (PRE_Y1) { dcg[j] += __shfl_xor(dcg[j], o); dcb[j] += __shfl_xor(dcb[j], o); dcs[j] += __shfl_xor(dcs[j], o); }
+      dg[j] += __shfl_xor(dg[j], o); db[j] += __shfl_xor(db[j], o);
+    }
+  float* red = reinterpret_cast<float*>(smem);
+  __syncthreads();
+  if (lane < 16) {
+#pragma unroll
+    for (int j = 0; j < 8; ++j) {
+      if constexpr (PRE_Y1) {
+        red[(0 * 4 + wave) * FD + lane * 8 + j] = dcg[j]; red[(1 * 4 + wave) * FD + lane * 8 + j] = dcb[j];
+        red[(2 * 4 + wave) * FD + lane * 8 + j] = dcs[j];
+      }
+      red[(3 * 4 + wave) * FD + lane * 8 + j] = dg[j]; red[(4 * 4 + wave) * FD + lane * 8 + j] = db[j];
+    }
+  }
+  __syncthreads();
+  for (int c = tid; c < 5 * FD; c += 256) {
+    const int q = c >> 7, n = c & (FD - 1);
+    const float* src = (!PRE_Y1 && q < 3) ? cacc : red;
+    a.partials[(size_t)blockIdx.x * 5 * FD + c] = (src[(q * 4 + 0) * FD + n] + src[(q * 4 + 1) * FD + n]) + (src[(q * 4 + 2) * FD + n] + src[(q * 4 + 3) * FD + n]);
+  }
+}
+
+__device__ __forceinline__ void acc_once(float* p, float v) {
+#if RG_DET
+  rg_acc(p, v);
+#else
+  *p += v;
+#endif
+}
+__global__ __launch_bounds__(256) void attn_out_bwd_cross_reduce_kernel(const float* __restrict__ partials, int nblocks, float* d0, float* d1,
+                                                                        float* d2, float* d3, float* d4) {
+  __shared__ float red[16][16];
+  const int col = threadIdx.x & 15, part = threadIdx.x >> 4, c = blockIdx.x * 16 + col;
+  const int q = c >> 7;
+  float* dst = q == 0 ? d0 : (q == 1 ? d1 : (q == 2 ? d2 : (q == 3 ? d3 : d4)));
+  float s0 = 0.f, s1 = 0.f;
+  int b = part;
+  for (; b + 16 < nblocks; b += 32) {
+    s0 += partials[(size_t)b * 5 * FD + c];
+    s1 += partials[(size_t)(b + 16) * 5 * FD + c];
+  }
+  if (b < nblocks) s0 += partials[(size_t)b * 5 * FD + c];
+  red[part][col] = s0 + s1;
+  __syncthreads();
+  if (part == 0 && dst) {
+    float t = 0.f;
+#pragma unroll
+    for (int r = 0; r < 16; ++r) t += red[r][col];
+    acc_once(dst + (c & (FD - 1)), t);
+  }
+}
+
+extern "C" size_t rg_attn_out_bwd_cross_workspace(int M) { return (size_t)(M <= 0 ? 0 : 512) * 5 * FD * sizeof(float); }
+
+extern "C" int rg_attn_out_bwd_cross(const rg_attn_out_bwd_cross_args* a, int dtype, void* stream) {
+  if (!a || a->M <= 0) return 0;
+  if (a->d != FD || a->P != FD) return rg_set_error_msg(RG_ERR_UNSUPPORTED, "attn_out_bwd_cross: needs d_model == n_heads*32 == 128");
+  if (!a->dy2 || !a->y2 || !a->rstd_c || !a->cgamma || !a->cbeta || !a->y1 || !a->rstd1 || !a->gamma1 || !a->beta1 || !a->Wot || !a->dy1
+      || !a->dz || !a->dctx || !a->partials)
+    return rg_set_error_msg(RG_ERR_INVALID, "attn_out_bwd_cross: NULL operand");
+  if ((long long)a->M * FD * 4 >= (1ll << 32)) return rg_set_error_msg(RG_ERR_UNSUPPORTED, "attn_out_bwd_cross: M too large for 32-bit offsets");
+  hipStream_t s = (hipStream_t)stream;
+  const int smem = 2 * act_tile_bytes(dtype, FT_M) + 6 * FD * 4 + (dtype == RG_BF16 ? 0 : 12 * FD * 4);
+  const int grid = attn_out_bwd_grid(a->M);
+  if (dtype == RG_BF16) {
+    hipFuncSetAttribute(reinterpret_cast<const void*>(attn_out_bwd_cross_kernel<__bf16>), hipFuncAttributeMaxDynamicSharedMemorySize, smem);
+    hipLaunchKernelGGL((attn_out_bwd_cross_kernel<__bf16>), dim3(grid), dim3(256), smem, s, *a);
+  } else if (dtype == RG_F32) {
+    hipFuncSetAttribute(reinterpret_cast<const void*>(attn_out_bwd_cross_kernel<float>), hipFuncAttributeMaxDynamicSharedMemorySize, smem);
+    hipLaunchKernelGGL((attn_out_bwd_cross_kernel<float>), dim3(grid), dim3(256), smem, s, *a);
+  } else if (dtype == RG_X3) {
+    hipFuncSetAttribute(reinterpret_cast<const void*>(attn_out_bwd_cross_kernel<x3>), hipFuncAttributeMaxDynamicSharedMemorySize, smem);
+    hipLaunchKernelGGL((attn_out_bwd_cross_kernel<x3>), dim3(grid), dim3(256), smem, s, *a);
+  } else return rg_set_error_msg(RG_ERR_INVALID, "attn_out_bwd_cross: bad dtype");
+  if (a->dcgamma || a->dcbeta || a->dz_colsum || a->dgamma1 || a->dbeta1)
+    hipLaunchKernelGGL(attn_out_bwd_cross_reduce_kernel, dim3(5 * FD / 16), dim3(256), 0, s, a->partials, grid, a->dcgamma, a->dcbeta, a->dz_colsum,
+                       a->dgamma1, a->dbeta1);
+  RG_CHECK_LAUNCH();
+  return 0;
+}
diff --git a/recguru_amd/hip.py b/recguru_amd/hip.py
--- a/recguru_amd/hip.py
+++ b/recguru_amd/hip.py
@@ -72,6 +72,14 @@
                 ("M", c_i), ("d", c_i), ("P", c_i), ("w_packed", c_i), ("live16", c_p)]
 
 
+class AttnOutBwdCrossArgs(ctypes.Structure):
+    _fields_ = [("dy2", c_p), ("y2", c_p), ("rstd_c", c_p), ("cgamma", c_p), ("cbeta", c_p),
+                ("y1", c_p), ("rstd1", c_p), ("gamma1", c_p), ("beta1", c_p), ("rowmask", c_p), ("Wot", c_p),
+                ("dy1", c_p), ("dz", c_p), ("dctx", c_p),
+                ("dcgamma", c_p), ("dcbeta", c_p), ("dz_colsum", c_p), ("dgamma1", c_p), ("dbeta1", c_p), ("partials", c_p),
+                ("M", c_i), ("d", c_i), ("P", c_i), ("w_packed", c_i), ("live16", c_p)]
+
+
 SYMBOLS = ["rg_last_error", "rg_version", "rg_gemm_nt", "rg_gemm_tn", "rg_attn_fwd", "rg_attn_bwd",
            "rg_embed_pe_fwd", "rg_embed_pe_fwd_rows", "rg_embed_scatter_bwd", "rg_ln_bwd", "rg_bcast_add_ln", "rg_seq_sum", "rg_colsum",
            "rg_outer_posmask", "rg_interpolate", "rg_gp_penalty", "rg_sum", "rg_adam", "rg_cast",
@@ -82,7 +90,7 @@
            "rg_assemble_batch", "rg_sample_negatives", "rg_sample_negatives_alias", "rg_dropout", "rg_cross_rows", "rg_live_tiles",
            "rg_adam_multi_dev", "rg_disc_rows", "rg_disc_supported", "rg_attn_fwd_x_supported", "rg_pad_mask", "rg_last_rows",
            "rg_ffn_bwd_data", "rg_ffn_bwd_data_supported", "rg_ffn_bwd_ln_workspace", "rg_first_live",
-           "rg_attn_out_bwd", "rg_attn_out_bwd_workspace",
+           "rg_attn_out_bwd", "rg_attn_out_bwd_workspace", "rg_attn_out_bwd_cross", "rg_attn_out_bwd_cross_workspace",
            "rg_item_loss_train_supported", "rg_item_loss_train", "rg_item_loss_scatter_binned", "rg_scale_dev",
            "rg_attn_lastq_x_supported", "rg_attn_lastq_x_fwd", "rg_attn_lastq_x_bwd", "rg_attn_lastq_xf_fwd", "rg_attn_lastq_xf_bwd",
            "rg_embed_scatter_binned_workspace", "rg_embed_scatter_bwd_binned", "rg_embed_pe_fwd_split", "rg_mse",
@@ -650,11 +658,12 @@
     return xl, ml
 
 
-def seq_sum(x, B, L):
+def seq_sum(x, B, L, rowmask=None):
     N = x.shape[-1]
     assert x.is_contiguous()
+    assert rowmask is None or (rowmask.dtype == torch.float32 and rowmask.numel() == B * L and rowmask.is_contiguous())
     out = torch.empty(B, N, device=x.device, dtype=x.dtype)
-    _check(lib().rg_seq_sum(_vp(x), _vp(out), B, L, N, dt_of(x), _stream()), "rg_seq_sum")
+    _check(lib().rg_seq_sum(_vp(x), _vp(out), B, L, N, dt_of(x), _stream(), _vp(rowmask)), "rg_seq_sum")
     return out
 
 
@@ -684,11 +693,12 @@
     return s
 
 
-def seq_wsum(x, s, B, L, H):
+def seq_wsum(x, s, B, L, H, rowmask=None):
     N = x.shape[-1]
     assert x.is_contiguous() and s.is_contiguous()
+    assert rowmask is None or (rowmask.dtype == torch.float32 and rowmask.numel() == B * L and rowmask.is_contiguous())
     out = torch.empty(B, H, N, device=x.device, dtype=x.dtype)
-    _check(lib().rg_seq_wsum(_vp(x), _vp(s), _vp(out), B, L, H, N, dt_of(x), _stream()), "rg_seq_wsum")
+    _check(lib().rg_seq_wsum(_vp(x), _vp(s), _vp(out), B, L, H, N, dt_of(x), _stream(), _vp(rowmask)), "rg_seq_wsum")
     return out
 
 
@@ -1339,6 +1349,30 @@
     return dz, dctx
 
 
+@_det_accum(dcgamma="g", dcbeta="g", dz_colsum="g", dgamma1="g", dbeta1="g")
+def attn_out_bwd_cross(dy2, y2, rstd_c, cgamma, cbeta, y1, rstd1, gamma1, beta1, rowmask, dcgamma, dcbeta, dgamma1, dbeta1, Wot,
+                       dz_colsum=None, live=None, w_packed=False):
+    M, d = dy2.shape
+    P = d
+    assert dy2.is_contiguous() and y2.is_contiguous() and y1.is_contiguous() and dy2.dtype == y2.dtype == y1.dtype
+    assert y2.shape == dy2.shape and y1.shape == dy2.shape
+    dy1 = torch.empty_like(dy2)
+    dz = torch.empty_like(dy2)
+    dctx = torch.empty(M, P, device=dy2.device, dtype=dy2.dtype)
+    if POISON_UNWRITTEN and live is not None:
+        dy1.fill_(float("nan"))
+        dz.fill_(float("nan"))
+        dctx.fill_(float("nan"))
+    fn = lib().rg_attn_out_bwd_cross_workspace
+    fn.restype = ctypes.c_size_t
+    ws = _tn_workspace(dy2.device, int(fn(M)), "attn_out_cross_ln")
+    a = AttnOutBwdCrossArgs(_p(dy2), _p(y2), _p(rstd_c), _p(cgamma), _p(cbeta), _p(y1), _p(rstd1), _p(gamma1), _p(beta1), _p(rowmask),
+                            _p(Wot), _p(dy1), _p(dz), _p(dctx), _p(dcgamma), _p(dcbeta), _p(dz_colsum), _p(dgamma1), _p(dbeta1), _p(ws),
+                            M, d, P, 1 if w_packed else 0, _p(live))
+    _check(lib().rg_attn_out_bwd_cross(ctypes.byref(a), mt_of(dy2), _stream()), "rg_attn_out_bwd_cross")
+    return dy1, dz, dctx
+
+
 def ffn_bwd_data_supported(d, dff):
     return bool(lib().rg_ffn_bwd_data_supported(int(d), int(dff)))
 
@@ -1555,6 +1589,11 @@
     return "attn_out_bwd_kernel", 2.0 * M * d * d, 4 * M * d * _esize(dy) + M * 4
 
 
+def _work_attn_out_bwd_cross(dy2, y2, rstd_c, *a, **k):
+    M, d = dy2.shape
+    return "attn_out_bwd_cross_kernel", 2.0 * M * d * d, 6 * M * d * _esize(dy2) + 3 * M * 4
+
+
 def _work_ln_bwd(dy, y, rstd, *a, **k):
     M, N = dy.shape
     return "ln_bwd_kernel", 0.0, 3 * M * N * _esize(dy) + M * 4
@@ -1600,7 +1639,7 @@
             + (2 * n * d * _esize(h) if target_route else 0))
 
 
-_WORK = {"full_ce_fwd": _work_full_ce_fwd, "full_ce_dw": _work_full_ce_dw, "shared_ce_fwd": _work_shared_ce_fwd, "shared_ce_dw": _work_shared_ce_dw, "attn_out_bwd": _work_attn_out_bwd, "ln_bwd": _work_ln_bwd, "gemm_tn_layer": _work_gemm_tn_layer, "item_loss_scatter_binned": _work_item_loss_scatter, "attn_lastq_x_fwd": _work_lastq_x_fwd, "attn_lastq_x_bwd": _work_lastq_x_bwd, "item_loss_train": _work_item_loss_train,
+_WORK = {"full_ce_fwd": _work_full_ce_fwd, "full_ce_dw": _work_full_ce_dw, "shared_ce_fwd": _work_shared_ce_fwd, "shared_ce_dw": _work_shared_ce_dw, "attn_out_bwd": _work_attn_out_bwd, "attn_out_bwd_cross": _work_attn_out_bwd_cross, "ln_bwd": _work_ln_bwd, "gemm_tn_layer": _work_gemm_tn_layer, "item_loss_scatter_binned": _work_item_loss_scatter, "attn_lastq_x_fwd": _work_lastq_x_fwd, "attn_lastq_x_bwd": _work_lastq_x_bwd, "item_loss_train": _work_item_loss_train,
          "ffn_bwd_data": _work_ffn_bwd, "attn_fwd_x": _work_attn_fwd_x, "post_attn_fwd": _work_post_attn, "gemm_nt": _work_gemm_nt, "gemm_tn": _work_gemm_tn, "attn_fwd": _work_attn_fwd, "attn_bwd": _work_attn_bwd,
          "embed_pe_fwd": _work_embed_fwd, "item_loss_fwd": _work_item_loss, "item_loss_bwd": _work_item_loss}
 _PLAIN = ["dropout_", "cross_rows", "adam_multi", "adam_multi_dev", "adam_multi_dev2", "grad_sqnorm_multi", "disc_rows", "item_loss_bwd_binned", "embed_scatter_bwd", "bcast_add_ln", "seq_sum", "colsum", "outer_posmask", "interpolate",
diff --git a/recguru_amd/ops.py b/recguru_amd/ops.py
--- a/recguru_amd/ops.py
+++ b/recguru_amd/ops.py
@@ -523,6 +523,7 @@
 EMBED_SCATTER_BINNED = True
 FUSE_ITEM_LOSS_TRAIN = True
 FUSE_ATTN_OUT_BWD = True
+FUSE_ATTN_OUT_BWD_CROSS = True
 LASTQ_FROM_X = True
 LASTQ_FOLD_PREFIX = True
 ATTN_RESIDENT_MAX_L = 416
@@ -593,6 +594,16 @@
         dz = hip.ln_bwd(dy, y, rstd, g.detach(), be.detach(), rowmask, dg, dbe, live=live)
         hip.gemm_tn(dz, ctx_.view(B * L, P), dWo, dbo, live=live if live is not None else _live_tn(rowmask, dz.shape[0], P, d))
         dctx = hip.gemm_nt(dz, shadow(Wo, transpose=True), live=live, skip_dead_fill=True)
+    dx, gqkv = _attn_block_bwd_qkv(dz, dctx, live, x2, saved, B, L, key_ids, pad_value, causal, H, prm, drop_p, seed, rowmask, x_masked)
+    return dx, gqkv + (rWo, rbo, rg, rbe)
+
+
+def _attn_block_bwd_qkv(dz, dctx, live, x2, saved, B, L, key_ids, pad_value, causal, H, prm, drop_p=0.0, seed=0, rowmask=None,
+                        x_masked=False):
+    Wq, bq, Wk, bk, Wv, bv = prm[:6]
+    qkv, ctx_, lse, _ = saved
+    d = x2.shape[1]
+    P = prm[6].shape[1]
     sub = (QKV_BIAS_ROWS_IN_ATTENTION and x_masked == 2 and _unwritten_qkv_ok() and L <= ATTN_RESIDENT_MAX_L
            and _zero_rows_live(rowmask, x2.shape[0], True, d, 3 * P) is not None)
     dqkv = hip.attn_bwd(qkv if qkv.dim() == 5 else qkv.view(B, L, -1), dctx.view(B, L, P), ctx_, lse, key_ids, pad_value, causal, H,
@@ -607,7 +618,7 @@
         dx = hip.gemm_nt(dqkv2[:, 384:], Wt[:, 384:], epilogue=hip.EPI_ADD, aux=dx, out=dx, live=live)
     else:
         dx = hip.gemm_nt(dqkv2, Wt, epilogue=hip.EPI_ADD, aux=dz, live=live)
-    return dx, (rW[0], rb[0], rW[1], rb[1], rW[2], rb[2], rWo, rbo, rg, rbe)
+    return dx, (rW[0], rb[0], rW[1], rb[1], rW[2], rb[2])
 
 
 def _ffn_block_fwd(y, rowmask, W1, b1, W2, b2, g, be, drop_p=0.0, seed_h1=0, seed_out=0):
@@ -924,14 +935,25 @@
                                      drop_p, seeds[1], seeds[2])
             (dcg, rcg), (dcbe, rcbe) = _gt(cg), _gt(cbe)
             (dcWo, rcWo), (dcbo, rcbo) = _gt(cWo), _gt(cbo)
-            dy1 = hip.ln_bwd(dy2, y2, rstd_c, cg.detach(), cbe.detach(), rowmask, dcg, dcbe,
-                             dz_colsum=dcbo if s_cross is not None else None)
+            Wo, bo, g1, be1 = ctx.prm[6:10]
+            cross = FUSE_ATTN_OUT_BWD_CROSS and FUSE_ATTN_OUT_BWD and d == 128 and Wo.shape[1] == 128
+            if cross:
+                (dg1, rg1), (dbe1, rbe1) = _gt(g1), _gt(be1)
+                live = _live(rowmask, B * L)
+                dy1, dz, dctx = hip.attn_out_bwd_cross(dy2, y2, rstd_c, cg.detach(), cbe.detach(), y1, rstd1, g1.detach(), be1.detach(),
+                                                       rowmask, dcg, dcbe, dg1, dbe1, shadow(Wo, transpose=True, pack=True, split=True),
+                                                       dz_colsum=dcbo if s_cross is not None else None, live=live, w_packed=True)
+                rm = rowmask
+            else:
+                dy1 = hip.ln_bwd(dy2, y2, rstd_c, cg.detach(), cbe.detach(), rowmask, dcg, dcbe,
+                                 dz_colsum=dcbo if s_cross is not None else None)
+                rm = None
             if s_cross is None:
-                do = hip.seq_sum(dy1, B, L)
+                do = hip.seq_sum(dy1, B, L, rowmask=rm)
                 hip.gemm_tn(do, c, dcWo, dcbo)
                 dc = hip.gemm_nt(do, shadow(cWo, transpose=True))
             else:
-                doh = hip.seq_wsum(dy1, s_cross, B, L, H)
+                doh = hip.seq_wsum(dy1, s_cross, B, L, H, rowmask=rm)
                 eye = _head_eye(H, c)
                 cm = (c.view(B, 1, H, 32) * eye).view(B * H, P)
                 doh2 = doh.reshape(B * H, d)
@@ -941,8 +963,15 @@
             (dcWv, rcWv), (dcbv, rcbv) = _gt(cWv), _gt(cbv)
             hip.gemm_tn(dc, u, dcWv, dcbv)
             du = hip.gemm_nt(dc, shadow(cWv, transpose=True))
-            dx, ga = _attn_block_bwd(dy1, x2, y1, (qkv, ctx_, lse, rstd1), B, L, key_ids, 0, True, H,
-                                     ctx.prm[:10], drop_p, seeds[0], rowmask, xm)
+            if cross:
+                (dWo, rWo), (dbo, rbo) = _gt(Wo), _gt(bo)
+                _tn(dz, ctx_.view(B * L, Wo.shape[1]), dWo, dbo, live=live)
+                dx, ga = _attn_block_bwd_qkv(dz, dctx, live, x2, (qkv, ctx_, lse, rstd1), B, L, key_ids, 0, True, H,
+                                             ctx.prm[:10], drop_p, seeds[0], rowmask, xm)
+                ga = ga + (rWo, rbo, rg1, rbe1)
+            else:
+                dx, ga = _attn_block_bwd(dy1, x2, y1, (qkv, ctx_, lse, rstd1), B, L, key_ids, 0, True, H,
+                                         ctx.prm[:10], drop_p, seeds[0], rowmask, xm)
         return ((dx.view(B, L, d), du.to(ctx.u_dtype), None, None, None, None, None) + ga + (rcWv, rcbv, rcWo, rcbo, rcg, rcbe) + gf)
 
 
```

Result: faster. 877,700 user-sequences/sec (median of 6 runs) (+1.1%).
